# juanmc2005/diart

Measured on AMD Instinct MI355X. Metric: real-time-factor xRT streams/GPU @500ms step, higher is better.
Workload: dtype f16x3

## Files before the change

### diart_amd/build.py

```python
from __future__ import annotations

import os
import shutil
import subprocess
import sys
from concurrent.futures import ThreadPoolExecutor
from pathlib import Path

HERE = Path(__file__).resolve().parent
CSRC = HERE / "csrc"
LIB = HERE / "libdiart_amd.so"
LIB_EXPERIMENTS = HERE / "libdiart_amd_exp.so"
SOURCES = ["api.hip", "seg_api.hip", "xvec_api.hip", "kernel_api.hip", "ecapa_api.hip", "k_front.hip", "k_convgemm.hip", "k_gemm_f32.hip", "k_gemm_split.hip", "k_gemm_pre.hip",
           "k_mlp_head.hip", "k_conv_pool.hip", "k_lstm.hip", "k_lstm_mfma.hip", "k_pool.hip",
           "k_ecapa.hip", "ecm_api.hip", "k_ecapa_mel.hip", "sbx_api.hip", "titanet_api.hip", "k_titanet.hip", "sbr_api.hip", "k_sb_resnet.hip", "wespeaker_api.hip", "k_wespeaker.hip", "k_conv2d.hip", "k_resample.hip", "k_volume.hip", "k_rows_repeat.hip", "k_gather.hip", "resample_api.hip", "ring.hip", "cluster.cpp", "tail.cpp", "hostpool.cpp", "filebatch.cpp", "k_tune.hip", "k_tune_vad.hip", "k_tune_score.hip", "tune_score.cpp"]
EXPERIMENT_SOURCES = ["experiments/k_gemm_g2.hip", "experiments/k_gemm_g3.hip"]
ARCH = "gfx950"
EXTRA_FLAGS = {"k_lstm_mfma.hip": ["-fno-slp-vectorize"]}


def _hipcc() -> str:
    for cand in (os.environ.get("HIPCC"), shutil.which("hipcc"), "/opt/rocm/bin/hipcc"):
        if cand and Path(cand).exists():
            return cand
    raise RuntimeError("hipcc not found (set HIPCC)")


def _stale(out: Path, deps) -> bool:
    if not out.exists():
        return True
    t = out.stat().st_mtime
    return any(Path(d).stat().st_mtime > t for d in deps)


def build(force: bool = False, verbose: bool = False, experiments: bool = False) -> Path:
    hipcc = _hipcc()
    objdir = HERE / "build" / ("exp" if experiments else "ship")
    objdir.mkdir(parents=True, exist_ok=True)
    headers = [CSRC / "dz_common.h", CSRC / "dz_embed.h", CSRC / "dz_sincnet.h", CSRC / "hostpool.h", CSRC / "tune_core.h", CSRC / "clu_core.h", HERE.parent / "include" / "diart_amd.h",
               HERE.parent / "include" / "diart_amd_experiments.h"]
    flags = ["-O3", "-std=c++17", "-fPIC", f"--offload-arch={ARCH}", "-Wall", "-Wno-unused-function", f"-I{CSRC}"]
    sources, lib = list(SOURCES), LIB
    if experiments:
        flags.append("-DDZ_EXPERIMENTS")
        sources, lib = sources + EXPERIMENT_SOURCES, LIB_EXPERIMENTS

    def compile_one(src: str) -> Path:
        s = CSRC / src
        o = objdir / (s.stem + ".o")
        if force or _stale(o, [s, *headers]):
            cmd = [hipcc, *flags, *EXTRA_FLAGS.get(src, []), "-x", "hip", "-c", str(s), "-o", str(o)]
            r = subprocess.run(cmd, capture_output=True, text=True)
            if r.returncode != 0:
                raise RuntimeError(f"hipcc failed on {src}:\n{r.stderr}")
            if verbose and r.stderr.strip():
                print(r.stderr, file=sys.stderr)
        return o

    with ThreadPoolExecutor(max_workers=min(len(sources), os.cpu_count() or 4)) as ex:
        objs = list(ex.map(compile_one, sources))
    if force or _stale(lib, objs):
        cmd = [hipcc, "-shared", "-fPIC", f"--offload-arch={ARCH}", *map(str, objs), "-o", str(lib), "-lpthread"]
        r = subprocess.run(cmd, capture_output=True, text=True)
        if r.returncode != 0:
            raise RuntimeError(f"link failed:\n{r.stderr}")
    return lib


if __name__ == "__main__":
    print(build(force="--force" in sys.argv, verbose=True, experiments="--experiments" in sys.argv))
```

### diart_amd/csrc/dz_common.h

```cpp
#pragma once
#include <hip/hip_runtime.h>
#include <hip/hip_ext.h>
#include <stdint.h>
#include <stddef.h>
#include <mutex>
#include "../../include/diart_amd.h"

#ifdef DZ_EXPERIMENTS
#include <stdlib.h>
static inline const char* dz_exp_env(const char* name) { return getenv(name); }
#else
#define dz_exp_env(name) ((const char*)nullptr)
#endif
enum { DZ_OPT_F32_GEMM = 0, DZ_OPT_POOL_FUSE, DZ_OPT_PACK_CACHE, DZ_OPT_COUNT };
int dz_option(int id);

typedef float f32x4 __attribute__((ext_vector_type(4)));
typedef float f32x2 __attribute__((ext_vector_type(2)));

#define DZ_MFMA(a, b, c) __builtin_amdgcn_mfma_f32_16x16x4f32((a), (b), (c), 0, 0, 0)

#define DZ_LEAKY_SLOPE 0.01f

struct DzAttrOnce {
    std::mutex mu;
    bool done[64] = {};
    hipError_t raise(const void* fn, int bytes) {
        int d = 0;
        (void)hipGetDevice(&d);
        std::lock_guard<std::mutex> lk(mu);
        if (d >= 0 && d < 64 && done[d]) return hipSuccess;
        const hipError_t e = hipFuncSetAttribute(fn, hipFuncAttributeMaxDynamicSharedMemorySize, bytes);
        if (e == hipSuccess && d >= 0 && d < 64) done[d] = true;
        return e;
    }
};

struct DzLaunchProf {
    hipEvent_t start, stop;
};
struct DzProfScope {
    DzProfScope(int tag, int units);
    ~DzProfScope();
};
enum DzProfTag {
    DZ_T_WAVE = 0, DZ_T_CONV0, DZ_T_FIN, DZ_T_CONV1, DZ_T_CONV2, DZ_T_PROJ, DZ_T_REC, DZ_T_MLP, DZ_T_CLS,
    DZ_T_TDNN1, DZ_T_TDNN2, DZ_T_TDNN3, DZ_T_TDNN4, DZ_T_TDNN5, DZ_T_POOL, DZ_T_EMBLIN, DZ_T_L2, DZ_T_OSP, DZ_T_PSET,
    DZ_T_CDIST, DZ_T_PROJ0,
    DZ_T_ECAPA_FBANK, DZ_T_ECAPA_BLOCK0, DZ_T_ECAPA_WIDE, DZ_T_ECAPA_RES2, DZ_T_ECAPA_SE, DZ_T_ECAPA_ASP, DZ_T_ECAPA_FC,
    DZ_T_CONV0_PAIR, DZ_T_NSPLIT, DZ_T_COUNT
};
extern thread_local int* dz_cur_oflag;
struct DzRangeScope {
    int* prev;
    explicit DzRangeScope(int* f) : prev(dz_cur_oflag) { dz_cur_oflag = f; }
    ~DzRangeScope() { dz_cur_oflag = prev; }
};
extern thread_local DzLaunchProf* dz_launch_prof;
#define DZ_LAUNCH(kernel, grid, block, lds, st, ...)                                          \
    do {                                                                                      \
        if (dz_launch_prof) {                                                                 \
            hipExtLaunchKernelGGL(kernel, grid, block, lds, st, dz_launch_prof->start,        \
                                  dz_launch_prof->stop, 0, __VA_ARGS__);                      \
            dz_launch_prof = nullptr;                             \
        } else {                                                                              \
            hipLaunchKernelGGL(kernel, grid, block, lds, st, __VA_ARGS__);                    \
        }                                                                                     \
    } while (0)

__device__ __forceinline__ void dz_tile_map_lin(int L, int gx, int gy, int gz, int agroup, int& bx, int& by,
                                                int& bz) {
    const int NA = gx * gz, NA8 = NA & ~7;
    int a;
    if (L < NA8 * gy) {
        const int xcd = L & 7, j = L >> 3;
        const int per = NA8 >> 3;
        const int AG = agroup > 0 ? agroup : 4;
        const int g = j / (AG * gy), r = j - g * (AG * gy);
        const int gsz = per - g * AG < AG ? per - g * AG : AG;
        by = r / gsz;
        a = (g * AG + (r - by * gsz)) * 8 + xcd;
    } else {
        const int r = L - NA8 * gy;
        a = NA8 + r / gy;
        by = r - (r / gy) * gy;
    }
    bz = a / gx;
    bx = a - bz * gx;
}
__device__ __forceinline__ void dz_tile_map(int agroup, int& bx, int& by, int& bz) {
    const int gx = gridDim.x, gy = gridDim.y;
    dz_tile_map_lin(blockIdx.x + gx * (blockIdx.y + gy * blockIdx.z), gx, gy, gridDim.z, agroup, bx, by, bz);
}

__device__ __forceinline__ int dz_xcd_contiguous(int b, int grid) {
    return (grid & 7) == 0 ? (b & 7) * (grid >> 3) + (b >> 3) : b;
}

__host__ __device__ __forceinline__ long long dz_kb(long long row, int col, long long R) {
    return ((long long)(col >> 5) * R + row) * 32 + (col & 31);
}

__device__ __forceinline__ unsigned short* dz_split_base(void* ysplit, long long yplane, bool odd) {
    unsigned short* y = reinterpret_cast<unsigned short*>(ysplit);
    return odd ? y + (yplane - 1) : y;
}
__device__ __forceinline__ void dz_store_split(unsigned short* ypl, long long idx, float v, bool store,
                                               bool odd, float& amax) {
    amax = fmaxf(amax, fabsf(v));
    const float x = __builtin_amdgcn_fmed3f(v, -65504.f, 65504.f);
    const _Float16 h = (_Float16)x;
    const _Float16 lw = (_Float16)((x - (float)h) * 2048.f);
    const unsigned P = (unsigned)__builtin_bit_cast(unsigned short, h) |
                       ((unsigned)__builtin_bit_cast(unsigned short, lw) << 16);
    const unsigned Q = (unsigned)__builtin_amdgcn_update_dpp(0, (int)P, 0xB1, 0xF, 0xF, true);
    const unsigned word = odd ? ((Q >> 16) | (P & 0xffff0000u)) : ((P & 0xffffu) | (Q << 16));
    if (store) *reinterpret_cast<unsigned*>(ypl + idx) = word;
}

__device__ __forceinline__ void dz_norm_from_partials(const float* __restrict__ partials, int b, int ntile,
                                                      int C, int T, const float* __restrict__ gamma,
                                                      const float* __restrict__ beta, float* out, int tid,
                                                      int nthreads, double* scratch) {
    const int G = nthreads / C > 0 ? nthreads / C : 1;
    const int c = tid % C, g = tid / C;
    if (g < G) {
        double s = 0.0, ss = 0.0;
        const float2* pp = reinterpret_cast<const float2*>(partials) + ((long long)b * ntile * C + c);
        int t = g;
        for (; t + 3 * G < ntile; t += 4 * G) {
            const float2 a0 = pp[(long long)t * C], a1 = pp[(long long)(t + G) * C];
            const float2 a2 = pp[(long long)(t + 2 * G) * C], a3 = pp[(long long)(t + 3 * G) * C];
            s += (double)a0.x; ss += (double)a0.y;
            s += (double)a1.x; ss += (double)a1.y;
            s += (double)a2.x; ss += (double)a2.y;
            s += (double)a3.x; ss += (double)a3.y;
        }
        for (; t < ntile; t += G) {
            const float2 a = pp[(long long)t * C];
            s += (double)a.x; ss += (double)a.y;
        }
        scratch[(g * C + c) * 2] = s;
        scratch[(g * C + c) * 2 + 1] = ss;
    }
    __syncthreads();
    if (tid < C) {
        double s = 0.0, ss = 0.0;
        for (int k = 0; k < G; ++k) {
            s += scratch[(k * C + tid) * 2];
            ss += scratch[(k * C + tid) * 2 + 1];
        }
        const double mean = s / T;
        double var = ss / T - mean * mean;
        if (var < 0.0) var = 0.0;
        const double rstd = 1.0 / sqrt(var + 1e-5);
        const double sc = (double)gamma[tid] * rstd;
        out[tid] = (float)sc;
        out[C + tid] = (float)((double)beta[tid] - mean * sc);
    }
}

__device__ __forceinline__ void dz_flag_range(int* oflag, float amax) {
    if (oflag && amax > 65504.f) *oflag = 1;
}

void dz_set_error(const char* fmt, ...);
#define DZ_HIP(expr)                                                                     \
    do {                                                                                 \
        hipError_t _e = (expr);                                                          \
        if (_e != hipSuccess) {                                                          \
            dz_set_error("%s failed: %s (%s:%d)", #expr, hipGetErrorString(_e), __FILE__, \
                         __LINE__);                                                      \
            return 1;                                                                    \
        }                                                                                \
    } while (0)
#define DZ_REQUIRE(cond, ...)           \
    do {                                \
        if (!(cond)) {                  \
            dz_set_error(__VA_ARGS__);  \
            return 2;                   \
        }                               \
    } while (0)

struct Arena {
    char* base = nullptr;
    size_t used = 0;
    template <typename T = float>
    T* take(size_t n) {
        const size_t bytes = (n * sizeof(T) + 255) & ~size_t(255);
        T* p = base ? reinterpret_cast<T*>(base + used) : nullptr;
        used += bytes;
        return p;
    }
};

template <typename H>
int dz_arena_alloc(const char* who, H* h, void (*carve)(H*, Arena&)) {
    Arena a;
    carve(h, a);
    const hipError_t err = hipMalloc((void**)&h->arena, a.used);
    if (err != hipSuccess) {
        h->arena = nullptr;
        dz_set_error("%s: hipMalloc(%zu) failed: %s", who, a.used, hipGetErrorString(err));
        return 1;
    }
    DZ_HIP(hipMemset(h->arena, 0, a.used));
    a.base = h->arena;
    a.used = 0;
    carve(h, a);
    return 0;
}

inline int dz_check_rows_forward(const char* who, const void* h, int max_rows, const float* d_wave, long long wave_stride,
                                 const float* d_masks, int n, int mask_frames, const float* d_out,
                                 const char* frames = "mask_frames") {
    DZ_REQUIRE(h && d_wave && d_out, "%s: NULL argument", who);
    DZ_REQUIRE(n >= 1 && n <= max_rows, "%s: %d rows outside [1, %d]", who, n, max_rows);
    DZ_REQUIRE(d_masks == nullptr || mask_frames >= 1, "%s: %s %d", who, frames, mask_frames);
    DZ_REQUIRE(wave_stride >= 0, "%s: negative stride", who);
    return 0;
}
inline int dz_check_groups_forward(const char* who, const void* h, int max_rows, const float* d_wave,
                                   long long wave_stride, const float* d_masks, int n_groups, int rows_per_group,
                                   int mask_frames, const float* d_out) {
    DZ_REQUIRE(h && d_wave && d_masks && d_out, "%s: NULL argument", who);
    DZ_REQUIRE(n_groups >= 1 && rows_per_group >= 1 && (long long)n_groups * rows_per_group <= max_rows,
               "%s: %d groups x %d rows outside [1, %d]", who, n_groups, rows_per_group, max_rows);
    DZ_REQUIRE(mask_frames >= 1, "%s: mask_frames %d", who, mask_frames);
    DZ_REQUIRE(wave_stride >= 0, "%s: negative stride", who);
    return 0;
}

struct DzRowGeometry {
    int S, Tc, min_samples, hop;
    long long lstride;
    float* sig;
    int *lens, *nvalid, *nmask, *tooshort;
    int *tdev, *rep_nvalid, *rep_nmask, *rep_T;
    void init(int num_samples, int min_num_samples, int hop = 160, int window = 400);
    void carve(Arena& a, size_t rows);
    int prologue(const float* d_wave, long long wave_stride, const float* d_masks, int mask_frames, int G, int K,
                 int rows_per_wave, hipStream_t st);
};

#define DZ_WS_G 8
__device__ __forceinline__ bool dz_ws_bad(const float* __restrict__ mom, int b) {
    const unsigned* m = reinterpret_cast<const unsigned*>(mom) + (long long)b * 2 * DZ_WS_G;
    bool bad = false;
#pragma unroll
    for (int i = 0; i < DZ_WS_G; ++i) bad |= (m[2 * i] & 0x7f800000u) == 0x7f800000u;
    return bad;
}
#ifdef DZ_EXPERIMENTS
extern long long* dz_conv_pool_dbg;
#endif
int dz_launch_wave_stats(const float* wave, long long stride, int B, int S, float* mom,
                         hipStream_t st);
int dz_launch_wave_stats_combine(const float* mom, int B, int S, float* stats, hipStream_t st);
int dz_launch_sinc_conv0(const float* wave, long long stride, int B, int S, const float* stats,
                         int stats_are_moments, float gamma, float beta, const float* filt,
                         float* y0, int P0, float* partials, int ntile, hipStream_t st);
int dz_launch_sinc_conv0_split(const float* wave, long long stride, int B, int S, const float* stats,
                               int stats_are_moments, float gamma, float beta, const void* filt_split,
                               float* y0, int P0, float* partials, int ntile, hipStream_t st, const void* ffrag = nullptr);
int dz_sinc_bank_frag_bytes();
int dz_launch_sinc_bank_frag(const void* fsp, void* frag, hipStream_t st);
int dz_conv0_split_ntile(int F0);
int dz_launch_sinc_conv0_pair(const float* wave, long long stride, int B, int S, const float* moments,
                              const void* pair_planes, const float* pair_bsum, float gamma_seg, float gamma_emb,
                              float* y0_seg, float* y0_emb, int P0, float* part_seg, float* part_emb, int ntile,
                              hipStream_t st);
int dz_launch_finalize_norm(const float* partials, int B, int ntile, int C, int T,
                            const float* gamma, const float* beta, float* scale, float* shift,
                            hipStream_t st);

typedef dz_convgemm_desc DzConvGemm;
constexpr int DZ_EPI_TG = 0x100;
int dz_launch_convgemm(const DzConvGemm& p, hipStream_t st);
bool dz_gemm_f32_ok(const DzConvGemm& p);
int dz_launch_gemm_f32(const DzConvGemm& p, hipStream_t st);
int dz_launch_gemm_split(const DzConvGemm& p, hipStream_t st);
int dz_launch_norm_f32(const float* y, const float* part, int ntile, int P, const float* gamma, const float* beta,
                       float* out, int B, hipStream_t st);
int dz_launch_norm_split(const float* y, const float* part, int ntile, int P, const float* gamma, const float* beta,
                         void* planes, long long plane, int B, hipStream_t st);
int dz_launch_conv_pool(const DzConvGemm& p, hipStream_t st, const void* wfrag = nullptr);
int dz_conv_pool_wfrag_bytes(int Cin);
int dz_launch_conv_pool_wfrag(int Cin, const void* wsplit, int Kpad, void* out, hipStream_t st);
int dz_launch_gemm_pre(const DzConvGemm& p, hipStream_t st);
#ifdef DZ_EXPERIMENTS
int dz_launch_gemm_g2(const DzConvGemm& p, int mt, hipStream_t st);
int dz_g2_default_mt();
#endif
int dz_gemm_gen();
#ifdef DZ_EXPERIMENTS
int dz_launch_gemm_g3(const DzConvGemm& p, int mt, hipStream_t st);
int dz_g3_error(int reset);
#endif
__device__ __forceinline__ float dz_pool_weight(const float* wr, int Fw, int T, int t) {
    const int F = Fw < 0 ? -Fw : Fw;
    if (F == T) return wr[t];
    const float scale = (float)F / (float)T;
    if (Fw < 0) {
        int i = (int)floorf((float)t * scale);
        if (i > F - 1) i = F - 1;
        return wr[i];
    }
    float src = scale * ((float)t + 0.5f) - 0.5f;
    if (src < 0.f) src = 0.f;
    const int i0 = (int)src;
    const int i1 = i0 + (i0 < F - 1 ? 1 : 0);
    const float l1 = src - (float)i0;
    return (1.f - l1) * wr[i0] + l1 * wr[i1];
}

struct DzPoolFuse {
    const float* w;
    int Fw, K;
    int P, T;
    int np;
    float* part;
    float* s0;
};
inline int dz_pool_pieces(int P) { return (P + 2 * 128 - 2) / 128; }
bool dz_gemm_pre_pool_ok(const DzConvGemm& p);
int dz_launch_gemm_pre_pool(const DzConvGemm& p, const DzPoolFuse& q, hipStream_t st);
int dz_launch_pool_combine(const float* part, const float* s0, int nx, int K, int np, int P, int T, int C,
                           int Npad, float* out, int ldo, hipStream_t st);
int dz_convgemm_ntile(int Tout);

int dz_launch_lstm(const float* gx, const float* whh, float* hout, void* hsplit, long long hplane,
                   int B, int T, int unit_major, hipStream_t st);
int dz_launch_lstm_mfma(const float* gx, const void* whh_split, float* hout, void* hsplit,
                        long long hplane, int B, int T, int unit_major, int variant, hipStream_t st);

int dz_launch_stats_pool(const float* X, long long xstride, int T, int C, int ldx,
                         const float* weights, int Fw, int rows, int rows_per_x, float* out, int ldo,
                         hipStream_t st);
int dz_launch_osp(const float* seg, int B, int F, int K, float gamma, float beta, int normalize,
                  int speaker_major, float* out, hipStream_t st);
__device__ __forceinline__ float dz_powg(float x, float gamma) {
    if (gamma == 3.f) return (x * x) * x;
    if (gamma == 2.f) return x * x;
    if (gamma == 1.f) return x;
    return powf(x, gamma);
}
__device__ __forceinline__ void dz_seg_decide(const float* lg, int classes, int K, int powerset, float* s) {
    if (powerset) {
        int best = 0;
        float bv = lg[0];
        for (int c = 1; c < classes; ++c)
            if (lg[c] > bv) {
                bv = lg[c];
                best = c;
            }
        int a = -1, b2 = -1;
        if (best >= 1 && best <= K) {
            a = best - 1;
        } else if (best > K) {
            int idx = best - K - 1;
            for (int i = 0; i < K && a < 0; ++i) {
                const int cnt = K - 1 - i;
                if (idx < cnt) {
                    a = i;
                    b2 = i + 1 + idx;
                } else {
                    idx -= cnt;
                }
            }
        }
        for (int k = 0; k < K; ++k) s[k] = (k == a || k == b2) ? 1.f : 0.f;
    } else {
        for (int k = 0; k < K; ++k) s[k] = 1.f / (1.f + expf(-lg[k]));
    }
}
__device__ __forceinline__ float dz_vad_frame(const float* s, int K) {
    float m = s[0];
    for (int k = 1; k < K; ++k) m = (s[k] > m || s[k] != s[k]) ? s[k] : m;
    return m;
}
__device__ __forceinline__ void dz_osp_frame(const float* s, int K, float gamma, float beta, float* w) {
    float e[8], m = -INFINITY;
    for (int k = 0; k < K; ++k) m = fmaxf(m, beta * s[k]);
    float sum = 0.f;
    for (int k = 0; k < K; ++k) {
        e[k] = expf(beta * s[k] - m);
        sum += e[k];
    }
    for (int k = 0; k < K; ++k) {
        const float pr = e[k] / sum;
        float wv = dz_powg(s[k], gamma) * dz_powg(pr, gamma);
        if (wv < 1e-8f) wv = 1e-8f;
        w[k] = wv;
    }
}

int dz_launch_seg_head(const float* m1, const float* cw, const float* cb, int B, int F, int classes, int K,
                       int powerset, float* seg, float gamma, float beta, int normalize, float* wout,
                       hipStream_t st, const float* wave_mom = nullptr, float* vad = nullptr);
struct DzMlpHead {
    const void* Xsplit;
    long long xplane;
    const void *W0split, *W1split;
    const float *b0, *b1, *cw, *cb;
    int rows, F, classes, K, powerset;
    float gamma, beta;
    float* seg;
    float* wout;
    int* oflag;
    const float* wave_mom;
    float* vad;
};
int dz_launch_mlp_head(const DzMlpHead& p, hipStream_t st);
int dz_launch_l2norm(float* x, int rows, int dim, float norm, hipStream_t st);
int dz_launch_splitk_finish(const float* parts, int nsplit, long long stride, int rows, int dim,
                            int normalize, float* out, hipStream_t st, const float* wave_mom = nullptr,
                            int rows_per_x = 1);
int dz_launch_powerset(const float* logp, int rows, int classes, int speakers, float* out,
                       hipStream_t st);
int dz_launch_cdist(const float* emb, const double* centers, int n, int k, int g, int dim,
                    double* out, hipStream_t st);

int dz_launch_mask_compact(const float* wave, long long stride, int S, const float* masks, int Fw,
                           int rows, float* sig, long long sig_stride, int* lens, hipStream_t st,
                           int rows_per_wave = 1);
int dz_launch_ecapa_geometry(const int* lens, int G, int K, int Tc, int min_samples, int hop, int* nvalid,
                             int* nmask, int* tooshort, int* tdev, int* rv, int* rm, int* rt, hipStream_t st);
int dz_launch_power(const float* spec, int lds, int bins, long long rows, float* pw, hipStream_t st);
int dz_launch_fbank_post(const float* melp, int n_mels, int T, int rows, const int* nvalid, float* feats,
                         hipStream_t st, const int* tdev = nullptr);
int dz_launch_se_mean(const float* x, int T, int C, int ldx, int rows, const int* nmask, float* s,
                      hipStream_t st);
int dz_launch_se_apply(const float* x, int ldx, const float* gate, const float* resid, int ldr,
                       float* out, int ldo, int rows, int T, int C, hipStream_t st);
int dz_launch_se_apply_planes(const float* x, int ldx, const float* gate, const float* resid, int ldr, float* out,
                              int ldo, void* planes, long long plane, int rows, int T, int C, hipStream_t st);
int dz_launch_asp_gstats(const float* x, int T, int C, int rows, const int* nmask, float* g,
                         hipStream_t st);
int dz_launch_asp_pool(const float* x, const float* logit, int T, int C, int rows, const int* nmask,
                       float* pooled, hipStream_t st);
int dz_launch_nan_rows(float* out, int rows, int dim, const int* flags, hipStream_t st);
int dz_launch_sb_stats_pool(const float* x, int T, int C, int ldx, int rows, const int* nvalid, float mean_bias,
                            float std_bias, float* pooled, hipStream_t st);

int dz_launch_ecm_prep(const float* sig, long long sig_stride, const int* lens, int rows, int K, float* csig,
                       long long cstride, int* lmax_out, hipStream_t st);
int dz_launch_ecm_magnitude(const float* spec, long long rows, float* mag, hipStream_t st);
int dz_launch_ecm_post(const float* melp, int T, int rows, const int* nvalid, float* feats, hipStream_t st);

struct DzConv2d {
    const float* X;
    const float* W;
    const void* Wsplit;
    const float* bias;
    const float* R;
    float* Y;
    int B, Fi, Ti, Cin, Fo, To, Cout, taps, stride, relu;
    int* oflag;
    const int* ext;
};
inline DzConv2d dz_conv2d(const float* W, const void* Wsplit, const float* bias, const float* X, int B, int Fi, int Ti,
                          int Cin, int Cout, int taps, int stride, const float* R, int relu, const int* ext, float* Y) {
    DzConv2d p = {};
    p.X = X; p.W = W; p.Wsplit = Wsplit; p.bias = bias; p.R = R; p.Y = Y; p.ext = ext;
    p.B = B; p.Fi = Fi; p.Ti = Ti; p.Cin = Cin; p.Cout = Cout; p.taps = taps; p.stride = stride; p.relu = relu;
    p.Fo = stride >= 1 ? (Fi - 1) / stride + 1 : 0;
    p.To = stride >= 1 ? (Ti - 1) / stride + 1 : 0;
    return p;
}
int dz_launch_conv2d(const DzConv2d& p, hipStream_t st);

enum { DZ_SBR_SE_SLICES = 16 };
int dz_launch_sbr_extents(const int* tdev, int rows, int s0, int s1, int s2, int s3, int* ext, hipStream_t st);
int dz_launch_sbr_stem(const float* feats, int rows, int Tb, int F, int C, const float* w, const float* b,
                       const int* ext, float* y, hipStream_t st);
int dz_launch_sbr_se_sum(const float* y, int rows, int Tb, int F, int C, const int* ext, float* part, hipStream_t st);
int dz_launch_sbr_se_fc(const float* part, int rows, int F, int C, int Cr, const int* ext, const float* w1t,
                        const float* b1, const float* w2t, const float* b2, float* gate, hipStream_t st);
int dz_launch_sbr_se_apply(const float* y, const float* gate, const float* r, int rows, int Tb, int F, int C,
                           const int* ext, float* out, hipStream_t st);
int dz_launch_sbr_att_pool(const float* x, const float* logits, int ldl, int rows, int Tb, int C, const int* ext,
                           float* pooled, hipStream_t st);

int dz_launch_wsp_fbank(const float* wave, long long stride, int N, int T, const float* mel, float* raw, int* bad,
                        hipStream_t st);
int dz_launch_wsp_cmn(const float* raw, int N, int T, const int* bad, float* feats, hipStream_t st);
int dz_launch_wsp_conv1(const float* feats, int N, int T, const float* w, const float* b, float* y, hipStream_t st);
int dz_launch_wsp_pool(const float* x, int B, int T4, const float* weights, int Fw, int K, const int* bad,
                       float* out, int* rflag, hipStream_t st);

int dz_launch_resample(const float* in, long long in_stride, long long in_len, int rows, const float* table,
                       int tap_major, int n, int n_pad, int o, int width, int T, float* out, long long out_stride,
                       long long out_len, hipStream_t st);

int dz_launch_rows_repeat(const float* wave, long long stride, int n_rows, int S, int* differs, int* repeat_out,
                          hipStream_t st);

struct dz_ctx {
    int device;
    int* oflag_host;
    int* oflag_dev;
    void* conv0_frag;
    void* convp_frag;
    const void* conv0_src;
    const void* convp_src;
    int convp_cin, convp_kpad;
    std::mutex frag_mu;
    hipStream_t conv0_user, convp_user;
    bool conv0_used, convp_used;
    int* rr_flags;
    int rr_cap;
    int* rr_host;
    int* rr_dev;
    std::mutex rr_mu;
    hipStream_t rr_user;
    bool rr_dirty;
};
```

### diart_amd/csrc/dz_embed.h

```cpp
#pragma once
#include "dz_common.h"

#include <string.h>
#include <new>

inline bool dz_conv_pool_enabled() {
    const char* v = dz_exp_env("DZ_CONV_POOL");
    return !(v && v[0] == '0');
}

struct DzGemm {
    DzConvGemm p;
    const void *wsplit, *wfrag;
    int tag, units;

    static DzGemm dense(const dz_layer& L, const float* X, int ldx, long long rows, int Cin, float* Y, int ldy,
                        int Nstore, int epi) {
        return conv1d(L, X, ldx, 1, (int)rows, Cin, Y, ldy, Nstore, epi).xstride(0, 0);
    }
    static DzGemm conv1d(const dz_layer& L, const float* X, int ldx, int B, int T, int Cin, float* Y, int ldy,
                         int Nstore, int epi) {
        DzGemm g;
        memset(&g, 0, sizeof(g));
        g.wsplit = L.wsplit;
        g.tag = -1;
        DzConvGemm& p = g.p;
        p.X = X; p.W = L.w; p.bias = L.b; p.e0 = L.s; p.e1 = L.h; p.Y = Y;
        p.B = B; p.Tin = p.Tout = p.Tstore = T; p.Cin = Cin; p.taps = 1; p.dil = 1; p.K = p.Kpad = Cin;
        p.Npad = p.Nstore = Nstore; p.ldx = ldx; p.ldy = ldy; p.epi = epi;
        return g.xstride((long long)T * ldx, (long long)T * ldy);
    }
    DzGemm& xstride(long long xbs, long long ybs) { p.xbs = xbs; p.ybs = ybs; return *this; }
    DzGemm& taps(int n, int dil, int pad) {
        p.taps = n; p.dil = dil; p.pad = pad; p.K = n * p.Cin;
        p.Tout = p.Tstore = pad ? p.Tin : p.Tin - (n - 1) * dil;
        return *this;
    }
    DzGemm& padded(int Kpad, int Npad) { p.Kpad = Kpad; p.Npad = Npad; return *this; }
    DzGemm& x2(const float* X2) { p.X2 = X2; return *this; }
    DzGemm& rowbias(const float* rb) { p.rowbias = rb; return *this; }
    DzGemm& splitk(int n, long long ysplit) { p.ksplit = n; p.ysplit = ysplit; return *this; }
    DzGemm& xplanes(const void* Xs, long long xplane) { p.Xsplit = Xs; p.xplane = Xs ? xplane : 0; return *this; }
    DzGemm& planes_out(void* Ys, long long yplane) { p.Ysplit = Ys; p.yplane = Ys ? yplane : 0; return *this; }
    DzGemm& norm_partials(const float* part, int tiles, int T, const float* gamma, const float* beta, int nld) {
        p.npart = part; p.npart_tiles = tiles; p.npart_T = T; p.ngamma = gamma; p.nbeta = beta;
        p.nld = nld; p.norm_on_load = 1;
        return *this;
    }
    DzGemm& norm_scaled(const float* nscale, const float* nshift, int nld) {
        p.nscale = nscale; p.nshift = nshift; p.nld = nld; p.norm_on_load = 1;
        return *this;
    }
    DzGemm& pool3(float* partials) {
        p.partials = partials; p.Tstore = p.Tout / 3; p.ybs = (long long)p.Tstore * p.ldy;
        return *this;
    }
    DzGemm& frag(const void* f) { wfrag = f; return *this; }
    DzGemm& tdev(const int* T) { p.Tdev = T; return *this; }
    DzGemm& prof(int t, int u) { tag = t; units = u; return *this; }

    int run(hipStream_t st) {
        DzProfScope ps(tag, units);
        if (p.Xsplit) {
            p.X = p.W = nullptr;
            p.Wsplit = wsplit;
            return dz_launch_gemm_pre(p, st);
        }
        if (wsplit && p.ksplit <= 1) {
            p.Wsplit = wsplit;
            if (p.epi == DZ_EPI_POOL3)
                return dz_conv_pool_enabled() ? dz_launch_conv_pool(p, st, wfrag) : dz_launch_gemm_split(p, st);
            p.Npad = (p.Npad + 127) / 128 * 128;
            return dz_launch_gemm_split(p, st);
        }
        DZ_REQUIRE(p.Ysplit == nullptr, "DzGemm: plane output asked of a layer that is not on the split-f16 path");
        return dz_launch_convgemm(p, st);
    }
    int run_pooled(const DzPoolFuse& q, hipStream_t st) {
        DzProfScope ps(tag, units);
        p.X = p.W = nullptr;
        p.Wsplit = wsplit;
        return dz_launch_gemm_pre_pool(p, q, st);
    }
};

constexpr int DZ_TAG_OF_GEMM = -2;
inline int dz_splitk_linear(const dz_layer& L, const float* X, int rows, int Cin, int Kpad, int N, int nsplit,
                            float* parts, int finish, float* out, hipStream_t st, int tag = -1,
                            int finish_tag = DZ_TAG_OF_GEMM, const float* wave_mom = nullptr, int rows_per_x = 1) {
    const long long ysplit = (long long)rows * N;
    if (int rc = DzGemm::dense(L, X, Cin, rows, Cin, parts, N, N, DZ_EPI_BIAS).padded(Kpad, N).splitk(nsplit, ysplit)
                     .prof(tag, rows / rows_per_x).run(st))
        return rc;
    DzProfScope ps(finish_tag == DZ_TAG_OF_GEMM ? tag : finish_tag, rows / rows_per_x);
    return dz_launch_splitk_finish(parts, nsplit, ysplit, rows, N, finish, out, st, wave_mom, rows_per_x);
}

inline int dz_fbank_front(const dz_layer& dft, const dz_layer& mel, const float* sig, long long lstride, int N, int T,
                          float* spec, float* pw, int nmel, int mel_npad, float* melp, hipStream_t st, int tag = -1) {
    const long long NT = (long long)N * T;
    int rc;
    if ((rc = DzGemm::conv1d(dft, sig, 160, N, T, 400, spec, 404, 402, DZ_EPI_BIAS).xstride(lstride, (long long)T * 404)
                  .padded(416, 448).prof(tag, N).run(st)))
        return rc;
    { DzProfScope ps(tag, N); if ((rc = dz_launch_power(spec, 404, 201, NT, pw, st))) return rc; }
    return DzGemm::dense(mel, pw, 204, NT, 204, melp, nmel, nmel, DZ_EPI_BIAS).padded(224, mel_npad).prof(tag, N).run(st);
}

struct DzAspTail {
    const float *wms, *zeros;
    const dz_layer *tdnn, *conv, *fc;
    float *gstat, *rb, *a1, *logits, *pooled, *parts;
    int nsplit, tag_asp, tag_fc;
};
inline int dz_asp_tail(const DzAspTail& a, const float* x, int N, int T, int C, int emb, const int* frames, float* out,
                       hipStream_t st) {
    int rc;
    { DzProfScope ps(a.tag_asp, N); if ((rc = dz_launch_asp_gstats(x, T, C, N, frames, a.gstat, st))) return rc; }
    const dz_layer wms = {a.wms, a.zeros, nullptr, nullptr, nullptr};
    if ((rc = dz_splitk_linear(wms, a.gstat, N, 2 * C, 2 * C, 128, a.nsplit, a.parts, 0, a.rb, st, a.tag_asp))) return rc;
    if ((rc = DzGemm::conv1d(*a.tdnn, x, C, N, T, C, a.a1, 128, 128, DZ_EPI_RELU_BN_TANH).rowbias(a.rb)
                  .prof(a.tag_asp, N).run(st)))
        return rc;
    if ((rc = DzGemm::dense(*a.conv, a.a1, 128, (long long)N * T, 128, a.logits, C, C, DZ_EPI_BIAS).prof(a.tag_asp, N)
                  .run(st)))
        return rc;
    { DzProfScope ps(a.tag_asp, N); if ((rc = dz_launch_asp_pool(x, a.logits, T, C, N, frames, a.pooled, st))) return rc; }
    return dz_splitk_linear(*a.fc, a.pooled, N, 2 * C, 2 * C, emb, a.nsplit, a.parts, 0, out, st, a.tag_fc);
}

struct DzEcapaTrunk {
    float *feats, *b0, *t1, *res, *t2, *cat, *mfa, *a1;
    float *smean, *sfc1, *gate, *gstat, *rb, *pooled, *parts;
    unsigned short *b0s, *ress, *cats;
    void carve(Arena& a, size_t N, size_t Tc, bool split);
    int run(const dz_ecapa_weights& w, int N, int T, const int* nmask, const int* tdev, float* d_out,
            hipStream_t st) const;
};

template <typename H>
int dz_handle_destroy(H* h) {
    if (h) {
        if (h->arena) (void)hipFree(h->arena);
        delete h;
    }
    return 0;
}
template <typename H, typename W>
int dz_handle_create(const char* who, dz_ctx* ctx, const W* w, int max_rows, int num_samples, int min_samples,
                     void (*carve)(H*, Arena&), H** out, int hop = 160, int window = 400) {
    DZ_REQUIRE(ctx && w && out, "%s: NULL argument", who);
    DZ_REQUIRE(max_rows >= 1 && num_samples >= min_samples, "%s: max_rows %d, %d samples", who, max_rows, num_samples);
    DZ_HIP(hipSetDevice(ctx->device));
    H* h = new (std::nothrow) H;
    DZ_REQUIRE(h != nullptr, "%s: out of memory", who);
    memset(h, 0, sizeof(*h));
    h->ctx = ctx; h->w = *w; h->Nm = max_rows;
    h->geo.init(num_samples, min_samples, hop, window);
    if (int rc = dz_arena_alloc(who, h, carve)) {
        dz_handle_destroy(h);
        return rc;
    }
    *out = h;
    return 0;
}
template <typename H, typename Run>
int dz_handle_forward(const char* who, H* h, const float* d_wave, long long wave_stride, const float* d_masks, int N,
                      int mask_frames, float* d_out, void* stream, Run run) {
    if (int rc = dz_check_rows_forward(who, h, h ? h->Nm : 0, d_wave, wave_stride, d_masks, N, mask_frames, d_out))
        return rc;
    DZ_HIP(hipSetDevice(h->ctx->device));
    DzRangeScope range_scope(h->ctx->oflag_dev);
    return run(h, d_wave, wave_stride, d_masks, 1, N, 1, mask_frames, 0, d_out, (hipStream_t)stream);
}
template <typename H, typename Run>
int dz_handle_forward_groups(const char* who, H* h, const float* d_wave, long long wave_stride, const float* d_masks,
                             int n_groups, int rows_per_group, int mask_frames, int normalize, float* d_out,
                             void* stream, Run run) {
    if (int rc = dz_check_groups_forward(who, h, h ? h->Nm : 0, d_wave, wave_stride, d_masks, n_groups, rows_per_group,
                                         mask_frames, d_out))
        return rc;
    DZ_HIP(hipSetDevice(h->ctx->device));
    DzRangeScope range_scope(h->ctx->oflag_dev);
    return run(h, d_wave, wave_stride, d_masks, n_groups, rows_per_group, rows_per_group, mask_frames, normalize, d_out,
               (hipStream_t)stream);
}
```

### diart_amd/csrc/k_gemm_pre.hip

```cpp
#include "dz_common.h"
#include <stdlib.h>
#include <type_traits>

namespace {

typedef _Float16 f16x8 __attribute__((ext_vector_type(8)));
typedef _Float16 f16x2 __attribute__((ext_vector_type(2)));
typedef float f32x16 __attribute__((ext_vector_type(16)));

constexpr int BM = 128, BN = 128, KT = 32;
constexpr int PLANE_B = 128 * 64;
constexpr int plane_a(int MW) { return 64 * MW * 64; }
constexpr int stage_bytes(int MW) { return 2 * plane_a(MW) + 2 * PLANE_B; }
constexpr size_t lds_bytes(int MW) { return 2 * (size_t)stage_bytes(MW) + 3 * BN * sizeof(float); }
constexpr int MW_BIG = 6;
constexpr float LO_UNSCALE = 1.f / 2048.f;

__device__ __forceinline__ float leaky(float v) { return fmaxf(v, v * DZ_LEAKY_SLOPE); }

constexpr int YT_PITCH = 132;
constexpr int POOL_PAR = BM * YT_PITCH * 4;
constexpr int POOL_WT = POOL_PAR + 3 * BN * 4;
constexpr int POOL_RED = POOL_WT + 4 * BM * 4;
constexpr int POOL_S0 = POOL_RED + 2 * 2 * 4 * BN * 4;
constexpr size_t POOL_LDS = POOL_S0 + 8 * 8 * 2 * 4 + 8 * 2 * 4;

template <int EPI, int MW, int MT, int NT, bool ILV = false, bool POOL = false>
__device__ __forceinline__ void gemm_pre_tile(const DzConvGemm& p, const int t0, const int n0, char* smem,
                                              const int flags = 0, const DzPoolFuse* q = nullptr) {
    constexpr int PLANE_A = plane_a(MW), STAGE = stage_bytes(MW), PAR_OFF = POOL ? POOL_PAR : 2 * STAGE;
    static_assert(!POOL || (MW == 2 && MT == 2 && NT == 2), "pooled epilogue: 128 x 128 tiles only");
    const int tid = threadIdx.x;
    const int w = __builtin_amdgcn_readfirstlane(tid >> 6), l = tid & 63;

    constexpr int PA = 2 * MT * MW, PB = 4 * NT, NWAVE = 2 * MW;
    constexpr int NWA = (NWAVE * PA + (PA + PB) / 2) / (PA + PB);
    constexpr int JMAX_A = (2 * PA + NWA - 1) / NWA, JMAX_B = (2 * PB + (NWAVE - NWA) - 1) / (NWAVE - NWA);
    constexpr int JMAX = JMAX_A > JMAX_B ? JMAX_A : JMAX_B;
    const bool isB = w >= NWA;
    const int rank = isB ? w - NWA : w, group = isB ? NWAVE - NWA : NWA, npc = isB ? PB : PA;
    const unsigned short* src = isB ? reinterpret_cast<const unsigned short*>(p.Wsplit)
                                    : reinterpret_cast<const unsigned short*>(p.Xsplit);
    const int prows = isB ? p.Npad : (int)((unsigned)p.xplane / (unsigned)p.ldx);
    const long long plane_el = isB ? (long long)p.Npad * p.Kpad : p.xplane;
    const unsigned nbytes = (unsigned)((long long)prows * (isB ? p.Kpad : p.ldx) * 2);
    const __amdgpu_buffer_rsrc_t rs_hi = __builtin_amdgcn_make_buffer_rsrc((void*)src, 0, nbytes, 0x00020000);
    const __amdgpu_buffer_rsrc_t rs_lo = __builtin_amdgcn_make_buffer_rsrc((void*)(src + plane_el), 0, nbytes, 0x00020000);
    const int voff0 = ((isB ? n0 : t0) + (l >> 2)) * 64 + (((l & 3) ^ ((l >> 4) & 3)) << 4);
    constexpr int vstep = 16 * 64;
    const int kb_bytes = prows * 64;
    const int dst0 = isB ? 2 * PLANE_A : 0, dplane = isB ? PLANE_B : PLANE_A;
    auto issue = [&](int kt, int stage) {
        int cblk = kt, tap = 0;
        if (p.taps > 1) {
            cblk = kt / p.taps;
            tap = kt - cblk * p.taps;
        }
        const int soff = isB ? (tap * (p.Cin >> 5) + cblk) * kb_bytes : cblk * kb_bytes + tap * p.dil * 64;
        char* dst = smem + stage * STAGE + dst0;
#pragma unroll
        for (int j = 0; j < JMAX; ++j) {
            const int q = rank + j * group;
            if (q >= 2 * npc) break;
            const int lo = q >= npc, i = q - lo * npc;
            __builtin_amdgcn_raw_ptr_buffer_load_lds(lo ? rs_lo : rs_hi,
                (__attribute__((address_space(3))) void*)(dst + lo * dplane + i * 1024), 16,
                voff0 + i * vstep, soff, 0, 0);
        }
    };

    const int li = l & 31, g = l >> 5;
    const int wm = w >> 1, wn = w & 1;
    const int sw = (li >> 2) & 3;
    int foff[2];
#pragma unroll
    for (int ks = 0; ks < 2; ++ks) foff[ks] = li * 64 + (((2 * ks + g) ^ sw) << 4);
    f32x16 accm[MT][NT], accx[MT][NT];
#pragma unroll
    for (int mt = 0; mt < MT; ++mt)
#pragma unroll
        for (int nt = 0; nt < NT; ++nt)
#pragma unroll
            for (int r = 0; r < 16; ++r) accm[mt][nt][r] = accx[mt][nt][r] = 0.f;

    auto compute = [&](int stage) {
        const char* st = smem + stage * STAGE;
        const char* sa = st + (wm * 32 * MT) * 64;
        const char* sb = st + 2 * PLANE_A + (wn * 32 * NT) * 64;
#pragma unroll
        for (int ks = 0; ks < 2; ++ks) {
            f16x8 ah[MT], al[MT], bh[NT], bl[NT];
#pragma unroll
            for (int t = 0; t < MT; ++t) {
                ah[t] = *reinterpret_cast<const f16x8*>(sa + t * 2048 + foff[ks]);
                al[t] = *reinterpret_cast<const f16x8*>(sa + PLANE_A + t * 2048 + foff[ks]);
            }
#pragma unroll
            for (int t = 0; t < NT; ++t) {
                bh[t] = *reinterpret_cast<const f16x8*>(sb + t * 2048 + foff[ks]);
                bl[t] = *reinterpret_cast<const f16x8*>(sb + PLANE_B + t * 2048 + foff[ks]);
            }
#pragma unroll
            for (int mt = 0; mt < MT; ++mt)
#pragma unroll
                for (int nt = 0; nt < NT; ++nt) {
                    accx[mt][nt] = __builtin_amdgcn_mfma_f32_32x32x16_f16(bh[nt], al[mt], accx[mt][nt], 0, 0, 0);
                    accm[mt][nt] = __builtin_amdgcn_mfma_f32_32x32x16_f16(bh[nt], ah[mt], accm[mt][nt], 0, 0, 0);
                    accx[mt][nt] = __builtin_amdgcn_mfma_f32_32x32x16_f16(bl[nt], ah[mt], accx[mt][nt], 0, 0, 0);
                }
        }
    };

    const int nk = p.Kpad / KT;
    issue(0, 0);
    constexpr bool FULL = MW == 2 && MT == 2 && NT == 2;
    float* par = reinterpret_cast<float*>(smem + PAR_OFF);
    {
        constexpr bool AFF = EPI == DZ_EPI_TDNN || EPI == DZ_EPI_RELU_BN;
        const int which = tid >> 5, c4 = (tid & 31) * 4;
        if (which < (AFF ? 3 : 1)) {
            const float* src = which == 0 ? p.bias : which == 1 ? p.e0 : p.e1;
            f32x4 v = {0.f, 0.f, 0.f, 0.f};
            if (n0 + c4 + 3 < p.Npad) v = *reinterpret_cast<const f32x4*>(src + n0 + c4);
            *reinterpret_cast<f32x4*>(par + which * BN + c4) = v;
        }
    }
    if (FULL && ILV) {
        const int r2 = w & 1;
        char* const dbase = smem + dst0 + r2 * 1024;
        const int vofs = voff0 + r2 * vstep;
        int cblk = 0, tap = 0;
        const int tap_step = isB ? (p.Cin >> 5) * kb_bytes : p.dil * 64;
        auto advance = [&]() -> int {
            if (++tap == p.taps) { tap = 0; ++cblk; }
            return cblk * kb_bytes + tap * tap_step;
        };
        int soff_next = 0, stage_next = 0;
        const bool no_dma = flags & 2, no_rd = flags & 4;
        const bool skip_a = (flags & 32) && !isB;
        auto piece = [&](int j) {
            const int lo = j >= 4, i = r2 + 2 * (j & 3);
            (void)i;
            if (no_dma || (skip_a && tap != 0 && cblk > 0)) return;
            __builtin_amdgcn_raw_ptr_buffer_load_lds(lo ? rs_lo : rs_hi,
                (__attribute__((address_space(3))) void*)(dbase + stage_next * STAGE + lo * dplane + (j & 3) * 2048), 16,
                vofs + (j & 3) * 2 * vstep, soff_next, 0, 0);
        };
        const char* sa0 = smem + (wm * 64) * 64;
        const char* sb0 = smem + 2 * PLANE_A + (wn * 64) * 64;
#define DZ_RD(base, plane, t, ks) (*reinterpret_cast<const f16x8*>((no_rd ? smem : (base) + (plane) + (t) * 2048) + foff[ks]))
#define DZ_MM(mt, nt)                                                                                     \
    accx[mt][nt] = __builtin_amdgcn_mfma_f32_32x32x16_f16(bh[nt], al[mt], accx[mt][nt], 0, 0, 0);          \
    accm[mt][nt] = __builtin_amdgcn_mfma_f32_32x32x16_f16(bh[nt], ah[mt], accm[mt][nt], 0, 0, 0);          \
    accx[mt][nt] = __builtin_amdgcn_mfma_f32_32x32x16_f16(bl[nt], ah[mt], accx[mt][nt], 0, 0, 0)
#define DZ_PIN() __builtin_amdgcn_sched_barrier(0)
        auto body = [&](const int kt, auto more_c) {
            constexpr bool more = decltype(more_c)::value;
            asm volatile("s_waitcnt vmcnt(0) lgkmcnt(0)\n\ts_barrier" ::: "memory");
            soff_next = advance();
            stage_next = (kt + 1) & 1;
            const char* sa = sa0 + (kt & 1) * STAGE;
            const char* sb = sb0 + (kt & 1) * STAGE;
            f16x8 ah[2], al[2], bh[2], bl[2];
            bh[0] = DZ_RD(sb, 0, 0, 0); al[0] = DZ_RD(sa, PLANE_A, 0, 0); ah[0] = DZ_RD(sa, 0, 0, 0);
            bl[0] = DZ_RD(sb, PLANE_B, 0, 0);
            bh[1] = DZ_RD(sb, 0, 1, 0); bl[1] = DZ_RD(sb, PLANE_B, 1, 0);
            ah[1] = DZ_RD(sa, 0, 1, 0); al[1] = DZ_RD(sa, PLANE_A, 1, 0);
            DZ_PIN();
            accx[0][0] = __builtin_amdgcn_mfma_f32_32x32x16_f16(bh[0], al[0], accx[0][0], 0, 0, 0);
            accm[0][0] = __builtin_amdgcn_mfma_f32_32x32x16_f16(bh[0], ah[0], accm[0][0], 0, 0, 0);
            DZ_PIN();
            if (more) piece(0);
            DZ_PIN();
            accx[0][0] = __builtin_amdgcn_mfma_f32_32x32x16_f16(bl[0], ah[0], accx[0][0], 0, 0, 0);
            accx[0][1] = __builtin_amdgcn_mfma_f32_32x32x16_f16(bh[1], al[0], accx[0][1], 0, 0, 0);
            DZ_PIN();
            if (more) piece(1);
            DZ_PIN();
            accm[0][1] = __builtin_amdgcn_mfma_f32_32x32x16_f16(bh[1], ah[0], accm[0][1], 0, 0, 0);
            accx[0][1] = __builtin_amdgcn_mfma_f32_32x32x16_f16(bl[1], ah[0], accx[0][1], 0, 0, 0);
            DZ_PIN();
            if (more) piece(2);
            ah[0] = DZ_RD(sa, 0, 0, 1); al[0] = DZ_RD(sa, PLANE_A, 0, 1);
            DZ_PIN();
            accx[1][1] = __builtin_amdgcn_mfma_f32_32x32x16_f16(bh[1], al[1], accx[1][1], 0, 0, 0);
            accm[1][1] = __builtin_amdgcn_mfma_f32_32x32x16_f16(bh[1], ah[1], accm[1][1], 0, 0, 0);
            DZ_PIN();
            if (more) piece(3);
            DZ_PIN();
            accx[1][1] = __builtin_amdgcn_mfma_f32_32x32x16_f16(bl[1], ah[1], accx[1][1], 0, 0, 0);
            accx[1][0] = __builtin_amdgcn_mfma_f32_32x32x16_f16(bh[0], al[1], accx[1][0], 0, 0, 0);
            DZ_PIN();
            if (more) piece(4);
            bh[1] = DZ_RD(sb, 0, 1, 1); bl[1] = DZ_RD(sb, PLANE_B, 1, 1);
            DZ_PIN();
            accm[1][0] = __builtin_amdgcn_mfma_f32_32x32x16_f16(bh[0], ah[1], accm[1][0], 0, 0, 0);
            accx[1][0] = __builtin_amdgcn_mfma_f32_32x32x16_f16(bl[0], ah[1], accx[1][0], 0, 0, 0);
            DZ_PIN();
            if (more) piece(5);
            bh[0] = DZ_RD(sb, 0, 0, 1); bl[0] = DZ_RD(sb, PLANE_B, 0, 1);
            ah[1] = DZ_RD(sa, 0, 1, 1); al[1] = DZ_RD(sa, PLANE_A, 1, 1);
            DZ_PIN();
            accx[0][1] = __builtin_amdgcn_mfma_f32_32x32x16_f16(bh[1], al[0], accx[0][1], 0, 0, 0);
            accm[0][1] = __builtin_amdgcn_mfma_f32_32x32x16_f16(bh[1], ah[0], accm[0][1], 0, 0, 0);
            DZ_PIN();
            if (more) piece(6);
            DZ_PIN();
            accx[0][1] = __builtin_amdgcn_mfma_f32_32x32x16_f16(bl[1], ah[0], accx[0][1], 0, 0, 0);
            accx[0][0] = __builtin_amdgcn_mfma_f32_32x32x16_f16(bh[0], al[0], accx[0][0], 0, 0, 0);
            DZ_PIN();
            if (more) piece(7);
            DZ_PIN();
            accm[0][0] = __builtin_amdgcn_mfma_f32_32x32x16_f16(bh[0], ah[0], accm[0][0], 0, 0, 0);
            accx[0][0] = __builtin_amdgcn_mfma_f32_32x32x16_f16(bl[0], ah[0], accx[0][0], 0, 0, 0);
            DZ_MM(1, 0);
            DZ_MM(1, 1);
        };
        for (int kt = 0; kt + 1 < nk; ++kt) body(kt, std::true_type{});
        body(nk - 1, std::false_type{});
#undef DZ_RD
#undef DZ_MM
#undef DZ_PIN
    } else
    for (int kt = 0; kt < nk; ++kt) {
        asm volatile("s_waitcnt vmcnt(0) lgkmcnt(0)\n\ts_barrier" ::: "memory");
        if (kt + 1 < nk) issue(kt + 1, (kt + 1) & 1);
        compute(kt & 1);
    }

    typedef _Float16 f16x4 __attribute__((ext_vector_type(4)));
    unsigned short* Yhi = reinterpret_cast<unsigned short*>(p.Ysplit);
    const long long yrows = Yhi ? (long long)((unsigned)p.yplane / (unsigned)p.ldy) : 0;
    float amax = 0.f;
    float* yt = reinterpret_cast<float*>(smem);
    if (POOL) __syncthreads();
    if constexpr (!POOL) {
        const bool whole = n0 + 64 * NT <= p.Nstore;
        const long long ybytes = Yhi ? 2 * (long long)yrows * p.ldy : 4 * (long long)p.Tout * p.ldy;
        if (whole && (Yhi != nullptr) != (p.Y != nullptr) && ybytes < (1ll << 31) && !(flags & 64)) {
            const unsigned nrec = __builtin_amdgcn_readfirstlane((unsigned)ybytes);
            const __amdgpu_buffer_rsrc_t r0 = __builtin_amdgcn_make_buffer_rsrc(Yhi ? (void*)Yhi : (void*)p.Y, 0, nrec, 0x00020000);
            const __amdgpu_buffer_rsrc_t r1 = __builtin_amdgcn_make_buffer_rsrc(Yhi ? (void*)(Yhi + p.yplane) : (void*)p.Y, 0, nrec, 0x00020000);
            typedef unsigned u32x2 __attribute__((ext_vector_type(2)));
            typedef unsigned u32x4 __attribute__((ext_vector_type(4)));
            const float* parl = par + wn * 32 * NT + 4 * g;
            auto sweep = [&](auto kind_c) {
                constexpr int KIND = decltype(kind_c)::value;
                constexpr bool PL = KIND != 0;
                u32x2 ph = {0u, 0u}, pw = {0u, 0u};
#pragma unroll
            for (int mt = 0; mt < MT; ++mt) {
                const int t = t0 + wm * 32 * MT + mt * 32 + li;
                const bool ok = t < p.Tout;
                float am = 0.f;
                const int vo = !ok ? (int)0x80000000 : KIND == 2 ? t * 64 + 16 * g : KIND == 1 ? t * 64 + 8 * g : (t * p.ldy + 4 * g) * 4;
#pragma unroll
                for (int nt = 0; nt < NT; ++nt) {
                    const int cb = n0 + wn * 32 * NT + nt * 32;
                    const int so = __builtin_amdgcn_readfirstlane(PL ? (cb >> 5) * (int)yrows * 64 : cb * 4);
#pragma unroll
                    for (int k = 0; k < 4; ++k) {
                        asm volatile("" ::: "memory");
                        const float* pg = parl + nt * 32 + 8 * k;
                        const f32x4 bv = *reinterpret_cast<const f32x4*>(pg);
                        f32x4 e0 = {1.f, 1.f, 1.f, 1.f}, e1 = {0.f, 0.f, 0.f, 0.f};
                        if (EPI == DZ_EPI_TDNN || EPI == DZ_EPI_RELU_BN) {
                            e0 = *reinterpret_cast<const f32x4*>(pg + BN);
                            e1 = *reinterpret_cast<const f32x4*>(pg + 2 * BN);
                        }
                        f32x4 v;
#pragma unroll
                        for (int e = 0; e < 4; ++e) {
                            float x = (accm[mt][nt][4 * k + e] + accx[mt][nt][4 * k + e] * LO_UNSCALE) + bv[e];
                            if (EPI == DZ_EPI_BIAS_LEAKY) x = leaky(x);
                            if (EPI == DZ_EPI_TDNN) x = leaky(x) * e0[e] + e1[e];
                            if (EPI == DZ_EPI_RELU_BN) x = fmaxf(x, 0.f) * e0[e] + e1[e];
                            v[e] = x;
                        }
                        if constexpr (!PL) {
                            __builtin_amdgcn_raw_buffer_store_b128(__builtin_bit_cast(u32x4, v), r0, vo + 32 * k, so, 0);
                        } else {
#pragma unroll
                        for (int e = 0; e < 4; ++e) {
                            am = fmaxf(am, fabsf(v[e]));
                            v[e] = __builtin_amdgcn_fmed3f(v[e], -65504.f, 65504.f);
                        }
                        asm volatile("" : "+v"(am));
                        const f16x4 hi = __builtin_convertvector(v, f16x4);
                        const f16x4 lo = __builtin_convertvector((v - __builtin_convertvector(hi, f32x4)) * 2048.f, f16x4);
                        if constexpr (KIND == 1) {
                            __builtin_amdgcn_raw_buffer_store_b64(__builtin_bit_cast(u32x2, hi), r0, vo + 16 * k, so, 0);
                            __builtin_amdgcn_raw_buffer_store_b64(__builtin_bit_cast(u32x2, lo), r1, vo + 16 * k, so, 0);
                        } else if ((k & 1) == 0) {
                            ph = __builtin_bit_cast(u32x2, hi);
                            pw = __builtin_bit_cast(u32x2, lo);
                        } else {
                            const u32x2 ch = __builtin_bit_cast(u32x2, hi), cw = __builtin_bit_cast(u32x2, lo);
                            u32x4 oh, ow;
#pragma unroll
                            for (int d = 0; d < 2; ++d) {
                                const auto sh = __builtin_amdgcn_permlane32_swap(ph[d], ch[d], false, false);
                                const auto sw2 = __builtin_amdgcn_permlane32_swap(pw[d], cw[d], false, false);
                                oh[d] = sh[0]; oh[2 + d] = sh[1];
                                ow[d] = sw2[0]; ow[2 + d] = sw2[1];
                            }
                            __builtin_amdgcn_raw_buffer_store_b128(oh, r0, vo + 32 * (k >> 1), so, 0);
                            __builtin_amdgcn_raw_buffer_store_b128(ow, r1, vo + 32 * (k >> 1), so, 0);
                        }
                        }
                    }
                }
                if (ok) amax = fmaxf(amax, am);
            }
            };
            if (!Yhi) sweep(std::integral_constant<int, 0>{});
            else if (flags & 128) sweep(std::integral_constant<int, 1>{});
            else sweep(std::integral_constant<int, 2>{});
            dz_flag_range(p.oflag, amax);
            return;
        }
    }
#pragma unroll
    for (int mt = 0; mt < MT; ++mt) {
        const int t = t0 + wm * 32 * MT + mt * 32 + li;
        const bool ok = t < p.Tout;
#pragma unroll
        for (int nt = 0; nt < NT; ++nt)
#pragma unroll
            for (int k = 0; k < 4; ++k) {
                asm volatile("" ::: "memory");
                const int n = n0 + wn * 32 * NT + nt * 32 + 8 * k + 4 * g;
                const int nc = n - n0;
                const f32x4 bv = *reinterpret_cast<const f32x4*>(par + nc);
                f32x4 e0 = {1.f, 1.f, 1.f, 1.f}, e1 = {0.f, 0.f, 0.f, 0.f};
                if (EPI == DZ_EPI_TDNN || EPI == DZ_EPI_RELU_BN) {
                    e0 = *reinterpret_cast<const f32x4*>(par + BN + nc);
                    e1 = *reinterpret_cast<const f32x4*>(par + 2 * BN + nc);
                }
                f32x4 v;
#pragma unroll
                for (int e = 0; e < 4; ++e) {
                    float x = (accm[mt][nt][4 * k + e] + accx[mt][nt][4 * k + e] * LO_UNSCALE) + bv[e];
                    if (EPI == DZ_EPI_BIAS_LEAKY) x = leaky(x);
                    if (EPI == DZ_EPI_TDNN) x = leaky(x) * e0[e] + e1[e];
                    if (EPI == DZ_EPI_RELU_BN) x = fmaxf(x, 0.f) * e0[e] + e1[e];
                    v[e] = x;
                }
                if (POOL) {
                    if (!(flags & 16)) *reinterpret_cast<f32x4*>(yt + (t - t0) * YT_PITCH + nc) = v;
                    continue;
                }
                const long long idx = (long long)t * p.ldy + n;
                if (p.Y && ok) {
                    if (n + 3 < p.Nstore) {
                        *reinterpret_cast<f32x4*>(p.Y + idx) = v;
                    } else {
#pragma unroll
                        for (int e = 0; e < 4; ++e)
                            if (n + e < p.Nstore) p.Y[idx + e] = v[e];
                    }
                }
                if (Yhi) {
#pragma unroll
                    for (int e = 0; e < 4; ++e) {
                        if (n + e >= p.Nstore) v[e] = 0.f;
                        if (ok) amax = fmaxf(amax, fabsf(v[e]));
                        v[e] = __builtin_amdgcn_fmed3f(v[e], -65504.f, 65504.f);
                    }
                    const f16x4 hi = __builtin_convertvector(v, f16x4);
                    const f16x4 lo = __builtin_convertvector((v - __builtin_convertvector(hi, f32x4)) * 2048.f, f16x4);
                    if (ok) {
                        const long long kidx = dz_kb(t, n, yrows);
                        *reinterpret_cast<f16x4*>(Yhi + kidx) = hi;
                        *reinterpret_cast<f16x4*>(Yhi + p.yplane + kidx) = lo;
                    }
                }
            }
    }
    dz_flag_range(p.oflag, amax);
    if constexpr (POOL) {
        if (flags & 24) return;
        float* wt = reinterpret_cast<float*>(smem + POOL_WT);
        float* red = reinterpret_cast<float*>(smem + POOL_RED);
        float* s0t = reinterpret_cast<float*>(smem + POOL_S0);
        float* s0f = s0t + 8 * 8 * 2;
        const int K = q->K, P = q->P, T = q->T;
        for (int i = tid; i < 4 * BM; i += 256) {
            const int rl = i >> 2, k = i & 3, r = t0 + rl;
            const int b = r / P, t = r - b * P;
            float wv = 0.f;
            if (k < K && t < T && r < p.Tout) {
                wv = 1.f;
                if (q->w) wv = dz_pool_weight(q->w + (long long)(b * K + k) * (q->Fw < 0 ? -q->Fw : q->Fw), q->Fw, T, t);
            }
            wt[i] = wv;
        }
        __syncthreads();
        const int b0 = t0 / P;
        int rb = (b0 + 1) * P - t0;
        if (rb > BM) rb = BM;
        if (tid < 64) {
            const int pk = tid >> 3, sub = tid & 7, part = pk >> 2, k = pk & 3;
            float a = 0.f, a2 = 0.f;
            if (k < K) {
                const int lo = max(part ? rb : 0, 16 * sub), hi = min(part ? BM : rb, 16 * sub + 16);
                for (int r = lo; r < hi; ++r) {
                    const float wv = wt[4 * r + k];
                    a += wv;
                    a2 += wv * wv;
                }
            }
            s0t[(pk * 8 + sub) * 2] = a;
            s0t[(pk * 8 + sub) * 2 + 1] = a2;
        }
        __syncthreads();
        if (tid < 8) {
            float a = 0.f, a2 = 0.f;
            for (int sub = 0; sub < 8; ++sub) {
                a += s0t[(tid * 8 + sub) * 2];
                a2 += s0t[(tid * 8 + sub) * 2 + 1];
            }
            s0f[tid * 2] = a;
            s0f[tid * 2 + 1] = a2;
        }
        const int wv_ = tid >> 6, c2 = 2 * (tid & 63);
        const int nx = p.Tout / P;
        auto pool_part = [&](auto kk_tag, const int part) {
            constexpr int KK = decltype(kk_tag)::value;
            const int lo = max(part ? rb : 0, 32 * wv_), hi = min(part ? BM : rb, 32 * wv_ + 32);
            float S[KK][2];
#pragma unroll
            for (int k = 0; k < KK; ++k) S[k][0] = S[k][1] = 0.f;
#pragma unroll 4
            for (int r = lo; r < hi; ++r) {
                const f32x2 x = *reinterpret_cast<const f32x2*>(yt + r * YT_PITCH + c2);
                const f32x4 w4 = *reinterpret_cast<const f32x4*>(wt + 4 * r);
#pragma unroll
                for (int k = 0; k < KK; ++k) {
                    S[k][0] = __builtin_fmaf(w4[k], x[0], S[k][0]);
                    S[k][1] = __builtin_fmaf(w4[k], x[1], S[k][1]);
                }
            }
#pragma unroll
            for (int k = 0; k < KK; ++k)
                *reinterpret_cast<f32x2*>(red + (wv_ * 4 + k) * BN + c2) = (f32x2){S[k][0], S[k][1]};
            __syncthreads();
            float mean[KK][2];
#pragma unroll
            for (int k = 0; k < KK; ++k) {
                f32x2 a = {0.f, 0.f};
#pragma unroll
                for (int v = 0; v < 4; ++v) a += *reinterpret_cast<const f32x2*>(red + (v * 4 + k) * BN + c2);
                const float v1 = s0f[(part * 4 + k) * 2];
                mean[k][0] = v1 > 0.f ? a[0] / v1 : 0.f;
                mean[k][1] = v1 > 0.f ? a[1] / v1 : 0.f;
            }
            __syncthreads();
#pragma unroll
            for (int k = 0; k < KK; ++k) S[k][0] = S[k][1] = 0.f;
#pragma unroll 4
            for (int r = lo; r < hi; ++r) {
                const f32x2 x = *reinterpret_cast<const f32x2*>(yt + r * YT_PITCH + c2);
                const f32x4 w4 = *reinterpret_cast<const f32x4*>(wt + 4 * r);
#pragma unroll
                for (int k = 0; k < KK; ++k) {
                    const float d0 = x[0] - mean[k][0], d1 = x[1] - mean[k][1];
                    S[k][0] = __builtin_fmaf(w4[k] * d0, d0, S[k][0]);
                    S[k][1] = __builtin_fmaf(w4[k] * d1, d1, S[k][1]);
                }
            }
#pragma unroll
            for (int k = 0; k < KK; ++k)
                *reinterpret_cast<f32x2*>(red + (wv_ * 4 + k) * BN + c2) = (f32x2){S[k][0], S[k][1]};
            __syncthreads();
            const int b = b0 + part;
            if (wv_ == 0 && b < nx) {
                const int piece = t0 / BM - (b * P) / BM;
#pragma unroll
                for (int k = 0; k < KK; ++k) {
                    f32x2 m2 = {0.f, 0.f};
#pragma unroll
                    for (int v = 0; v < 4; ++v) m2 += *reinterpret_cast<const f32x2*>(red + (v * 4 + k) * BN + c2);
                    float* o = q->part + ((((long long)b * q->np + piece) * K + k) * p.Npad + n0 + c2) * 2;
                    *reinterpret_cast<f32x4*>(o) = (f32x4){mean[k][0], m2[0], mean[k][1], m2[1]};
                    if (n0 == 0 && c2 == 0) {
                        float* so = q->s0 + (((long long)b * q->np + piece) * K + k) * 2;
                        so[0] = s0f[(part * 4 + k) * 2];
                        so[1] = s0f[(part * 4 + k) * 2 + 1];
                    }
                }
            }
        };
        for (int part = 0; part < (rb < BM ? 2 : 1); ++part) {
            if (part) __syncthreads();
            switch (K) {
                case 1: pool_part(std::integral_constant<int, 1>{}, part); break;
                case 2: pool_part(std::integral_constant<int, 2>{}, part); break;
                case 3: pool_part(std::integral_constant<int, 3>{}, part); break;
                default: pool_part(std::integral_constant<int, 4>{}, part); break;
            }
        }
    }
}

template <int EPI, bool ILV>
__global__ __launch_bounds__(256, 2) void gemm_pre_kernel(DzConvGemm p, int mbig, int msmall, int flags) {
    extern __shared__ __attribute__((aligned(16))) char smem[];
#ifndef DZ_EXPERIMENTS
    flags = 0;
#endif
    const int gy = p.Npad / BN, L = blockIdx.x;
    if (L < mbig * gy) {
        int bx, by, bz;
        dz_tile_map_lin(L, mbig, gy, 1, p.agroup, bx, by, bz);
        gemm_pre_tile<EPI, 2, 2, 2, ILV>(p, bx * BM, by * BN, smem, flags);
    } else {
        const int Ls = L - mbig * gy, gys = 2 * gy;
        const int xcd = Ls & 7, j = Ls >> 3;
        const int ms = (j / gys) * 8 + xcd, by = j % gys;
        if (ms >= msmall) return;
        gemm_pre_tile<EPI, 2, 1, 1>(p, mbig * BM + ms * 64, by * 64, smem);
    }
}

__global__ __launch_bounds__(256, 2) void gemm_pre_pool_kernel(DzConvGemm p, DzPoolFuse q, int gx, int flags) {
    extern __shared__ __attribute__((aligned(16))) char smem[];
    const int gy = p.Npad / BN;
    int bx, by, bz;
    dz_tile_map_lin(blockIdx.x, gx, gy, 1, p.agroup, bx, by, bz);
#ifndef DZ_EXPERIMENTS
    flags = 0;
#endif
    gemm_pre_tile<DZ_EPI_TDNN, 2, 2, 2, true, true>(p, bx * BM, by * BN, smem, flags, &q);
}

template <int EPI>
__global__ __launch_bounds__(64 * 2 * MW_BIG) void gemm_pre_big_kernel(DzConvGemm p) {
    extern __shared__ __attribute__((aligned(16))) char smem[];
    const int gy = p.Npad / BN, gx = (p.Tout + 64 * MW_BIG - 1) / (64 * MW_BIG);
    int bx, by, bz;
    dz_tile_map_lin(blockIdx.x, gx, gy, 1, p.agroup, bx, by, bz);
    gemm_pre_tile<EPI, MW_BIG, 2, 2>(p, bx * 64 * MW_BIG, by * BN, smem);
}
int big_tiles_mode() {
    static const int mode = [] {
        const char* e = dz_exp_env("DZ_GEMM_BIG");
        return e ? atoi(e) : 0;
    }();
    return mode;
}

bool interleaved_loop() {
    static const bool on = [] {
        const char* e = dz_exp_env("DZ_GP_LOOP");
        return !(e && e[0] == '0');
    }();
    return on;
}

int dbg_flags() {
    static const int f = [] {
        const char* e = dz_exp_env("DZ_GP_DBG");
        return e ? atoi(e) : 0;
    }();
    return f;
}

bool tail_tiles_enabled() {
    static const bool on = [] {
        const char* e = dz_exp_env("DZ_GEMM_TAIL");
        return e && e[0] == '1';
    }();
    return on;
}
int wg_slots() {
    static const int slots = [] {
        int dev = 0, cus = 256;
        if (hipGetDevice(&dev) == hipSuccess) hipDeviceGetAttribute(&cus, hipDeviceAttributeMultiprocessorCount, dev);
        return 2 * (cus > 0 ? cus : 256);
    }();
    return slots;
}

template <int EPI>
int launch(const DzConvGemm& p, hipStream_t st) {
    static DzAttrOnce attr_ilv;
    DZ_HIP(attr_ilv.raise((const void*)gemm_pre_kernel<EPI, true>, (int)lds_bytes(2)));
    const int gx = (p.Tout + BM - 1) / BM, gy = p.Npad / BN, slots = wg_slots();
#ifdef DZ_EXPERIMENTS
    static DzAttrOnce attr_once, attr_big;
    DZ_HIP(attr_once.raise((const void*)gemm_pre_kernel<EPI, false>, (int)lds_bytes(2)));
    {
        const int gxb = (p.Tout + 64 * MW_BIG - 1) / (64 * MW_BIG);
        const int mode = big_tiles_mode();
        if (mode == 1 && gxb >= 8) {
            DZ_HIP(attr_big.raise((const void*)gemm_pre_big_kernel<EPI>, (int)lds_bytes(MW_BIG)));
            DZ_LAUNCH((gemm_pre_big_kernel<EPI>), dim3(gxb * gy), dim3(64 * 2 * MW_BIG), lds_bytes(MW_BIG), st, p);
            DZ_HIP(hipGetLastError());
            return 0;
        }
    }
#endif
    int mbig = gx;
    const int tiles = gx * gy, rem = tiles % slots;
    if (4 * tiles < slots)
        mbig = 0;
    else if (tail_tiles_enabled() && rem != 0 && 4 * rem < 3 * slots)
        mbig = (tiles / slots) * slots / gy;
    const int rows_left = p.Tout - mbig * BM;
    const int msmall = rows_left > 0 ? (rows_left + 63) / 64 : 0;
    const int nwg = mbig * gy + ((msmall + 7) / 8) * 8 * (2 * gy);
#ifdef DZ_EXPERIMENTS
    if (!interleaved_loop())
        DZ_LAUNCH((gemm_pre_kernel<EPI, false>), dim3(nwg), dim3(256), lds_bytes(2), st, p, mbig, msmall, 0);
    else
#endif
        DZ_LAUNCH((gemm_pre_kernel<EPI, true>), dim3(nwg), dim3(256), lds_bytes(2), st, p, mbig, msmall, dbg_flags());
    DZ_HIP(hipGetLastError());
    return 0;
}

}

int dz_gemm_gen() {
    static const int gen = [] {
        const char* e = dz_exp_env("DZ_GEMM_GEN");
        const int v = e ? atoi(e) : 1;
        return v == 2 || v == 3 ? v : 1;
    }();
    return gen;
}

bool dz_gemm_pre_pool_ok(const DzConvGemm& p) {
    const int gx = (p.Tout + BM - 1) / BM, gy = p.Npad / BN;
    return 4 * gx * gy >= wg_slots();
}

int dz_launch_gemm_pre_pool(const DzConvGemm& p_in, const DzPoolFuse& q, hipStream_t st) {
    DzConvGemm p = p_in;
    if (!p.oflag) p.oflag = dz_cur_oflag;
    DZ_REQUIRE(p.Wsplit && p.Xsplit && q.part && q.s0, "gemm_pre_pool: NULL operand");
    DZ_REQUIRE(p.epi == DZ_EPI_TDNN && p.B == 1 && p.taps == 1 && p.K == p.Kpad && p.Cin % KT == 0 &&
                   p.Npad % BN == 0 && p.Tout == p.Tin,
               "gemm_pre_pool: built for the flattened 1 x 1 TDNN layer");
    DZ_REQUIRE(q.np == dz_pool_pieces(q.P), "gemm_pre_pool: np must be dz_pool_pieces(P)");
    DZ_REQUIRE(q.K >= 1 && q.K <= 4 && q.P >= BM && q.T >= 2 && q.T <= q.P && p.Tout % q.P == 0 && (q.Fw >= 2 || q.Fw <= -2),
               "gemm_pre_pool: 1..4 speakers, chunk pitch >= 128 rows (got K %d, P %d, T %d)", q.K, q.P, q.T);
    DZ_REQUIRE(p.ldx > 0 && p.ldx % KT == 0 && p.xplane % p.ldx == 0 && p.xplane / p.ldx >= p.Tin,
               "gemm_pre_pool: kb-major input planes need ldx %% 32 == 0 and xplane = rows * ldx with rows >= Tin");
    DZ_REQUIRE(p.xplane * 2 < (1ll << 31) && (long long)p.Npad * p.Kpad * 2 < (1ll << 31),
               "gemm_pre_pool: operand plane exceeds the 2 GiB buffer-offset range");
    static const int pool_ag = [] {
        const char* e = dz_exp_env("DZ_POOL_AG");
        return e && atoi(e) > 0 ? atoi(e) : 1;
    }();
    if (!p.agroup) p.agroup = pool_ag;
    static DzAttrOnce attr_once;
    DZ_HIP(attr_once.raise((const void*)gemm_pre_pool_kernel, (int)POOL_LDS));
    const int gx = (p.Tout + BM - 1) / BM, gy = p.Npad / BN;
    DZ_LAUNCH(gemm_pre_pool_kernel, dim3(gx * gy), dim3(256), POOL_LDS, st, p, q, gx, dbg_flags());
    DZ_HIP(hipGetLastError());
    return 0;
}

int dz_launch_gemm_pre(const DzConvGemm& p_in, hipStream_t st) {
    DzConvGemm p = p_in;
    if (!p.oflag) p.oflag = dz_cur_oflag;
    DZ_REQUIRE(p.Wsplit != nullptr && p.Xsplit != nullptr,
               "gemm_pre: Wsplit / Xsplit (f16 hi/lo planes of W and of the input) are NULL");
    DZ_REQUIRE(p.Y != nullptr || p.Ysplit != nullptr, "gemm_pre: no output");
    DZ_REQUIRE(p.B == 1, "gemm_pre: flattened layers only (B = 1)");
    DZ_REQUIRE(p.K == p.Kpad && p.K == p.taps * p.Cin && p.Cin % KT == 0,
               "gemm_pre: K = taps * Cin without padding, Cin a multiple of 32");
    DZ_REQUIRE(p.Npad % BN == 0, "gemm_pre: Npad must be a multiple of 128");
    DZ_REQUIRE(p.Tout > 0 && p.Tout == p.Tin - (p.taps - 1) * p.dil, "gemm_pre: Tout mismatch");
    DZ_REQUIRE(p.pad == 0 && p.X2 == nullptr && p.rowbias == nullptr && p.ksplit <= 1 && !p.norm_on_load,
               "gemm_pre: padding / second input / row bias / split-K / norm-on-load are not built here");
    DZ_REQUIRE(p.ldx > 0 && p.ldx % KT == 0 && p.xplane % p.ldx == 0 && p.xplane / p.ldx >= p.Tin,
               "gemm_pre: kb-major input planes need ldx %% 32 == 0 and xplane = rows * ldx with rows >= Tin");
    DZ_REQUIRE(p.xplane * 2 < (1ll << 31) && (long long)p.Npad * p.Kpad * 2 < (1ll << 31),
               "gemm_pre: operand plane exceeds the 2 GiB buffer-offset range");
    DZ_REQUIRE(p.Ysplit == nullptr || (p.ldy > 0 && p.ldy % KT == 0 && p.yplane % p.ldy == 0 && p.yplane / p.ldy >= p.Tout &&
                                       p.Npad <= p.ldy && p.yplane * 2 < (1ll << 31)),
               "gemm_pre: kb-major output planes need ldy %% 32 == 0, yplane = rows * ldy with rows >= Tout, Npad <= ldy");
    DZ_REQUIRE(p.Y == nullptr || (p.ldy % 4 == 0 && ((uintptr_t)p.Y & 15) == 0),
               "gemm_pre: f32 output needs ldy a multiple of 4 and a 16-byte aligned base");
#ifdef DZ_EXPERIMENTS
    if (dz_gemm_gen() >= 2 && 4 * ((p.Tout + BM - 1) / BM) * (p.Npad / BN) >= wg_slots()) {
        static const int g3_min_k = [] {
            const char* e = dz_exp_env("DZ_G3_MINK");
            return e ? atoi(e) : 1024;
        }();
        if (dz_gemm_gen() == 3) {
            if (p.K >= g3_min_k) return dz_launch_gemm_g3(p, 0, st);
        } else {
            return dz_launch_gemm_g2(p, 0, st);
        }
    }
#endif
    switch (p.epi) {
        case DZ_EPI_BIAS: return launch<DZ_EPI_BIAS>(p, st);
        case DZ_EPI_BIAS_LEAKY: return launch<DZ_EPI_BIAS_LEAKY>(p, st);
        case DZ_EPI_TDNN: return launch<DZ_EPI_TDNN>(p, st);
        case DZ_EPI_RELU_BN: return launch<DZ_EPI_RELU_BN>(p, st);
    }
    dz_set_error("gemm_pre: epilogue %d is not built on the pre-split path", p.epi);
    return 2;
}
```

### diart_amd/csrc/kernel_api.hip

```cpp
#include "dz_sincnet.h"

extern "C" int dz_k_convgemm(dz_ctx* ctx, const dz_convgemm_desc* d, void* stream) {
    DZ_REQUIRE(ctx && d, "dz_k_convgemm: NULL argument");
    DZ_HIP(hipSetDevice(ctx->device));
    DzRangeScope range_scope(ctx->oflag_dev);
    return dz_launch_convgemm(*d, (hipStream_t)stream);
}
extern "C" int dz_k_gemm_f32(dz_ctx* ctx, const dz_convgemm_desc* d, void* stream) {
    DZ_REQUIRE(ctx && d, "dz_k_gemm_f32: NULL argument");
    DZ_HIP(hipSetDevice(ctx->device));
    return dz_launch_gemm_f32(*d, (hipStream_t)stream);
}
extern "C" int dz_k_gemm_split(dz_ctx* ctx, const dz_convgemm_desc* d, void* stream) {
    DZ_REQUIRE(ctx && d, "dz_k_gemm_split: NULL argument");
    DZ_HIP(hipSetDevice(ctx->device));
    DzRangeScope range_scope(ctx->oflag_dev);
    return dz_launch_gemm_split(*d, (hipStream_t)stream);
}
extern "C" int dz_k_gemm_pre(dz_ctx* ctx, const dz_convgemm_desc* d, void* stream) {
    DZ_REQUIRE(ctx && d, "dz_k_gemm_pre: NULL argument");
    DZ_HIP(hipSetDevice(ctx->device));
    DzRangeScope range_scope(ctx->oflag_dev);
    return dz_launch_gemm_pre(*d, (hipStream_t)stream);
}
#ifdef DZ_EXPERIMENTS
static int gemm_gen_open(const char* who, dz_ctx* ctx, const dz_convgemm_desc* d, DzConvGemm* p) {
    DZ_REQUIRE(ctx && d, "%s: NULL argument", who);
    DZ_REQUIRE(d->Wsplit && d->Xsplit && (d->Y || d->Ysplit) && d->B == 1 && d->K == d->Kpad && d->K == d->taps * d->Cin &&
                   d->Cin % 32 == 0 && d->Npad % 128 == 0 && d->pad == 0 && !d->X2 && !d->rowbias && d->ksplit <= 1 &&
                   !d->norm_on_load && d->Tout > 0 && d->Tout == d->Tin - (d->taps - 1) * d->dil && d->ldx % 32 == 0 &&
                   d->xplane % d->ldx == 0 && d->xplane / d->ldx >= d->Tin,
               "%s: the requirements of dz_k_gemm_pre apply", who);
    DZ_HIP(hipSetDevice(ctx->device));
    *p = *d;
    if (!p->oflag) p->oflag = ctx->oflag_dev;
    return 0;
}
extern "C" int dz_k_gemm_g2(dz_ctx* ctx, const dz_convgemm_desc* d, int row_fragments, void* stream) {
    DzConvGemm p;
    if (int rc = gemm_gen_open("dz_k_gemm_g2", ctx, d, &p)) return rc;
    DzRangeScope range_scope(ctx->oflag_dev);
    return dz_launch_gemm_g2(p, row_fragments, (hipStream_t)stream);
}
extern "C" int dz_k_gemm_g3(dz_ctx* ctx, const dz_convgemm_desc* d, int row_fragments, void* stream) {
    DzConvGemm p;
    if (int rc = gemm_gen_open("dz_k_gemm_g3", ctx, d, &p)) return rc;
    DzRangeScope range_scope(ctx->oflag_dev);
    return dz_launch_gemm_g3(p, row_fragments, (hipStream_t)stream);
}
#endif
extern "C" int dz_k_mlp_head(dz_ctx* ctx, const void* xsplit, long long xplane, const void* w0split,
                             const void* w1split, const float* b0, const float* b1, const float* cw,
                             const float* cb, int rows, int frames, int classes, int speakers, int powerset,
                             float gamma, float beta, float* d_seg, float* d_weights, void* stream) {
    DZ_REQUIRE(ctx, "dz_k_mlp_head: NULL argument");
    DZ_HIP(hipSetDevice(ctx->device));
    DzRangeScope range_scope(ctx->oflag_dev);
    DzMlpHead m{};
    m.Xsplit = xsplit; m.xplane = xplane; m.W0split = w0split; m.W1split = w1split;
    m.b0 = b0; m.b1 = b1; m.cw = cw; m.cb = cb;
    m.rows = rows; m.F = frames; m.classes = classes; m.K = speakers; m.powerset = powerset;
    m.gamma = gamma; m.beta = beta; m.seg = d_seg; m.wout = d_weights;
    return dz_launch_mlp_head(m, (hipStream_t)stream);
}
extern "C" int dz_k_seg_head(dz_ctx* ctx, const float* m1, const float* cw, const float* cb, int batch,
                             int frames, int classes, int speakers, int powerset, float* d_seg, float gamma,
                             float beta, int normalize, float* d_weights, void* stream) {
    DZ_REQUIRE(ctx && m1 && cw && cb && d_seg, "dz_k_seg_head: NULL argument");
    DZ_HIP(hipSetDevice(ctx->device));
    return dz_launch_seg_head(m1, cw, cb, batch, frames, classes, speakers, powerset, d_seg, gamma, beta,
                              normalize, d_weights, (hipStream_t)stream);
}
extern "C" int dz_k_conv_pool(dz_ctx* ctx, const dz_convgemm_desc* d, void* stream) {
    DZ_REQUIRE(ctx && d, "dz_k_conv_pool: NULL argument");
    DZ_HIP(hipSetDevice(ctx->device));
    DzRangeScope range_scope(ctx->oflag_dev);
    DZ_REQUIRE(d->Wsplit && (d->Cin == 80 || d->Cin == 64), "dz_k_conv_pool: Wsplit is NULL or Cin is not 80 / 64");
    std::lock_guard<std::mutex> frag_lock(ctx->frag_mu);
    if (!ctx->convp_frag) DZ_HIP(hipMalloc(&ctx->convp_frag, (size_t)dz_conv_pool_wfrag_bytes(80)));
    if (ctx->convp_used && ctx->convp_user != (hipStream_t)stream) DZ_HIP(hipStreamSynchronize(ctx->convp_user));
    ctx->convp_user = (hipStream_t)stream; ctx->convp_used = true;
    int rc;
    if (!(dz_option(DZ_OPT_PACK_CACHE) && ctx->convp_src == d->Wsplit && ctx->convp_cin == d->Cin && ctx->convp_kpad == d->Kpad)) {
        if ((rc = dz_launch_conv_pool_wfrag(d->Cin, d->Wsplit, d->Kpad, ctx->convp_frag, (hipStream_t)stream))) return rc;
        ctx->convp_src = d->Wsplit; ctx->convp_cin = d->Cin; ctx->convp_kpad = d->Kpad;
    }
    return dz_launch_conv_pool(*d, (hipStream_t)stream, ctx->convp_frag);
}
#ifdef DZ_EXPERIMENTS
extern "C" int dz_k_conv_pool_debug(long long* d_stamps) {
    dz_conv_pool_dbg = d_stamps;
    return 0;
}
#endif
extern "C" int dz_k_convgemm_ntile(int t_out) { return dz_convgemm_ntile(t_out); }
extern "C" int dz_k_wave_stats(dz_ctx* ctx, const float* d_wave, long long stride, int batch,
                               int samples, float* d_stats, void* stream) {
    DZ_REQUIRE(ctx && d_stats, "dz_k_wave_stats: NULL argument");
    int rc;
    if ((rc = check_wave("dz_k_wave_stats", d_wave, stride, samples))) return rc;
    DZ_HIP(hipSetDevice(ctx->device));
    float* mom = nullptr;
    DZ_HIP(hipMalloc((void**)&mom, (size_t)batch * 2 * DZ_WS_G * sizeof(float)));
    rc = dz_launch_wave_stats(d_wave, stride, batch, samples, mom, (hipStream_t)stream);
    if (!rc) rc = dz_launch_wave_stats_combine(mom, batch, samples, d_stats, (hipStream_t)stream);
    (void)hipStreamSynchronize((hipStream_t)stream);
    (void)hipFree(mom);
    return rc;
}
extern "C" int dz_k_sinc_conv0(dz_ctx* ctx, const float* d_wave, long long stride, int batch,
                               int samples, const float* d_stats, float gamma, float beta,
                               const float* d_filt, float* d_y0, float* d_partials, void* stream) {
    DZ_REQUIRE(ctx && d_stats && d_filt && d_y0 && d_partials, "dz_k_sinc_conv0: NULL argument");
    int rc;
    if ((rc = check_wave("dz_k_sinc_conv0", d_wave, stride, samples))) return rc;
    const SincGeom g = sinc_geom(samples);
    DZ_REQUIRE(g.P0 > 0, "dz_k_sinc_conv0: %d samples is too short", samples);
    DZ_HIP(hipSetDevice(ctx->device));
    return dz_launch_sinc_conv0(d_wave, stride, batch, samples, d_stats, 0, gamma, beta, d_filt, d_y0,
                                g.P0, d_partials, g.nt0, (hipStream_t)stream);
}
extern "C" int dz_k_sinc_conv0_split(dz_ctx* ctx, const float* d_wave, long long stride, int batch,
                                     int samples, const float* d_stats, float gamma, float beta,
                                     const void* d_filt_split, float* d_y0, float* d_partials,
                                     void* stream) {
    DZ_REQUIRE(ctx && d_stats && d_filt_split && d_y0 && d_partials, "dz_k_sinc_conv0_split: NULL argument");
    int rc;
    if ((rc = check_wave("dz_k_sinc_conv0_split", d_wave, stride, samples))) return rc;
    const SincGeom g = sinc_geom(samples, true);
    DZ_REQUIRE(g.P0 > 0, "dz_k_sinc_conv0_split: %d samples is too short", samples);
    DZ_HIP(hipSetDevice(ctx->device));
    DzRangeScope range_scope(ctx->oflag_dev);
    std::lock_guard<std::mutex> frag_lock(ctx->frag_mu);
    if (!ctx->conv0_frag) DZ_HIP(hipMalloc(&ctx->conv0_frag, (size_t)dz_sinc_bank_frag_bytes()));
    if (ctx->conv0_used && ctx->conv0_user != (hipStream_t)stream) DZ_HIP(hipStreamSynchronize(ctx->conv0_user));
    ctx->conv0_user = (hipStream_t)stream; ctx->conv0_used = true;
    if (!(dz_option(DZ_OPT_PACK_CACHE) && ctx->conv0_src == d_filt_split)) {
        if ((rc = dz_launch_sinc_bank_frag(d_filt_split, ctx->conv0_frag, (hipStream_t)stream))) return rc;
        ctx->conv0_src = d_filt_split;
    }
    return dz_launch_sinc_conv0_split(d_wave, stride, batch, samples, d_stats, 0, gamma, beta,
                                      d_filt_split, d_y0, g.P0, d_partials, g.nt0, (hipStream_t)stream, ctx->conv0_frag);
}
extern "C" int dz_k_conv0_split_ntile(int samples) { return sinc_geom(samples, true).nt0; }
#ifdef DZ_EXPERIMENTS
extern "C" int dz_k_sinc_conv0_pair(dz_ctx* ctx, const float* d_wave, long long stride, int batch, int samples,
                                    const float* d_moments, const void* d_pair_planes, const float* d_pair_bsum,
                                    float gamma_seg, float gamma_emb, float* d_y0_seg, float* d_y0_emb,
                                    float* d_part_seg, float* d_part_emb, void* stream) {
    DZ_REQUIRE(ctx && d_moments && d_pair_planes && d_pair_bsum && d_y0_seg && d_y0_emb && d_part_seg && d_part_emb,
               "dz_k_sinc_conv0_pair: NULL argument");
    const SincGeom g = sinc_geom(samples, true);
    DZ_REQUIRE(batch >= 1 && g.F0 >= 3, "dz_k_sinc_conv0_pair: empty input");
    int rc;
    if ((rc = check_wave("dz_k_sinc_conv0_pair", d_wave, stride, samples))) return rc;
    DZ_HIP(hipSetDevice(ctx->device));
    DzRangeScope range_scope(ctx->oflag_dev);
    return dz_launch_sinc_conv0_pair(d_wave, stride, batch, samples, d_moments, d_pair_planes, d_pair_bsum, gamma_seg,
                                     gamma_emb, d_y0_seg, d_y0_emb, g.P0, d_part_seg, d_part_emb, g.nt0,
                                     (hipStream_t)stream);
}
#endif
extern "C" int dz_k_finalize_norm(dz_ctx* ctx, const float* d_partials, int batch, int ntile,
                                  int channels, int frames, const float* d_gamma,
                                  const float* d_beta, float* d_scale, float* d_shift,
                                  void* stream) {
    DZ_REQUIRE(ctx && d_partials && d_gamma && d_beta && d_scale && d_shift,
               "dz_k_finalize_norm: NULL argument");
    DZ_HIP(hipSetDevice(ctx->device));
    return dz_launch_finalize_norm(d_partials, batch, ntile, channels, frames, d_gamma, d_beta,
                                   d_scale, d_shift, (hipStream_t)stream);
}
extern "C" int dz_k_lstm(dz_ctx* ctx, const float* d_gx, const float* d_whh, float* d_hout,
                         int batch, int frames, void* stream) {
    DZ_REQUIRE(ctx && d_gx && d_whh && d_hout, "dz_k_lstm: NULL argument");
    DZ_REQUIRE(batch >= 1 && frames >= 1, "dz_k_lstm: empty input");
    DZ_HIP(hipSetDevice(ctx->device));
    return dz_launch_lstm(d_gx, d_whh, d_hout, nullptr, 0, batch, frames, 0, (hipStream_t)stream);
}
extern "C" int dz_k_lstm_planes(dz_ctx* ctx, const float* d_gx, const float* d_whh,
                                const void* d_whh_split, int variant, void* d_hsplit, long long hplane,
                                int batch, int frames, void* stream) {
    DZ_REQUIRE(ctx && d_gx && d_hsplit && (d_whh || d_whh_split), "dz_k_lstm_planes: NULL argument");
    DZ_REQUIRE(batch >= 1 && frames >= 1, "dz_k_lstm_planes: empty input");
    DZ_HIP(hipSetDevice(ctx->device));
    if (d_whh_split)
        return dz_launch_lstm_mfma(d_gx, d_whh_split, nullptr, d_hsplit, hplane, batch, frames, variant >= 3 ? 1 : 0,
                                   variant, (hipStream_t)stream);
    return dz_launch_lstm(d_gx, d_whh, nullptr, d_hsplit, hplane, batch, frames, 0, (hipStream_t)stream);
}
extern "C" int dz_k_lstm_mfma(dz_ctx* ctx, const float* d_gx, const void* d_whh_split, float* d_hout,
                              int batch, int frames, int unit_major, int variant, void* stream) {
    DZ_REQUIRE(ctx && d_gx && d_whh_split && d_hout, "dz_k_lstm_mfma: NULL argument");
    DZ_REQUIRE(batch >= 1 && frames >= 1, "dz_k_lstm_mfma: empty input");
    DZ_HIP(hipSetDevice(ctx->device));
    return dz_launch_lstm_mfma(d_gx, d_whh_split, d_hout, nullptr, 0, batch, frames, unit_major,
                               variant, (hipStream_t)stream);
}
extern "C" int dz_k_stats_pool(dz_ctx* ctx, const float* d_x, int frames, int channels, int ldx,
                               const float* d_weights, int weight_frames, int rows,
                               int rows_per_x, float* d_out, int ldo, void* stream) {
    DZ_REQUIRE(ctx && d_x && d_out, "dz_k_stats_pool: NULL argument");
    DZ_REQUIRE(rows >= 1 && rows_per_x >= 1 && frames >= 2, "dz_k_stats_pool: empty input");
    DZ_HIP(hipSetDevice(ctx->device));
    DZ_REQUIRE(!d_weights || weight_frames >= 2 || weight_frames <= -2, "dz_k_stats_pool: weight_frames %d", weight_frames);
    return dz_launch_stats_pool(d_x, (long long)frames * ldx, frames, channels, ldx, d_weights,
                                d_weights ? weight_frames : frames, rows, rows_per_x, d_out, ldo,
                                (hipStream_t)stream);
}
extern "C" int dz_k_powerset(dz_ctx* ctx, const float* d_logits, int rows, int classes,
                             int speakers, float* d_out, void* stream) {
    DZ_REQUIRE(ctx && d_logits && d_out, "dz_k_powerset: NULL argument");
    DZ_HIP(hipSetDevice(ctx->device));
    return dz_launch_powerset(d_logits, rows, classes, speakers, d_out, (hipStream_t)stream);
}
```

### diart_amd/csrc/xvec_api.hip

```cpp
#include "dz_sincnet.h"

struct dz_emb {
    dz_ctx* ctx;
    dz_emb_weights w;
    SincGeom g;
    int Bm, T[5];
    bool pre;
    const float* ext_stats;
    const float* cur_stats;
    int ext_conv0_B;
    char* arena;
    SincScratch ss;
    float *a, *b, *x5, *pooled, *parts, *ppart, *ps0;
    int pending_B;
    const float* pending_in;
};
static const int kTdnnTaps[5] = {5, 3, 3, 1, 1};
static const int kTdnnDil[5] = {1, 2, 3, 1, 1};
static const int kTdnnCin[5] = {64, 512, 512, 512, 512};
static const int kTdnnN[5] = {512, 512, 512, 512, 1536};
static const int kPoolLd = 3008;
static const int kMaxSpk = 8;
static const int kEmbSplit = 16;

extern "C" int dz_emb_frames_for(int num_samples) {
    const int f = sinc_geom(num_samples).P2 - 4 - 4 - 6;
    return f > 0 ? f : 0;
}

static void emb_carve(dz_emb* e, Arena& a) {
    e->ss.carve(a, e->g, e->Bm);
    e->a = a.take((size_t)e->Bm * e->g.P2 * 512);
    e->b = a.take((size_t)e->Bm * e->g.P2 * 512);
    e->x5 = a.take((size_t)e->Bm * e->g.P2 * 1536);
    e->pooled = a.take((size_t)e->Bm * kMaxSpk * kPoolLd);
    const int np = dz_pool_pieces(e->g.P2);
    e->ppart = a.take((size_t)e->Bm * np * 4 * 1536 * 2);
    e->ps0 = a.take((size_t)e->Bm * np * 4 * 2);
    e->parts = a.take((size_t)kEmbSplit * e->Bm * kMaxSpk * 512);
}

extern "C" int dz_emb_create(dz_ctx* ctx, const dz_emb_weights* w, int max_batch, int num_samples,
                             dz_emb** out) {
    DZ_REQUIRE(ctx && w && out, "dz_emb_create: NULL argument");
    DZ_REQUIRE(max_batch >= 1, "dz_emb_create: max_batch %d", max_batch);
    DZ_REQUIRE(w->dimension == 512, "dz_emb_create: dimension %d (only 512 is built)", w->dimension);
    const SincGeom g = sinc_geom(num_samples, w->sinc.filt_split != nullptr);
    DZ_REQUIRE(g.ok && g.P2 > 14, "dz_emb_create: %d samples is too short", num_samples);
    DZ_REQUIRE((w->sinc.w1_split != nullptr) == (w->sinc.w2_split != nullptr) &&
                   (w->sinc.w1_split != nullptr) == (w->tw_split[0] != nullptr),
               "dz_emb_create: the split planes of SincNet conv1 / conv2 and of tdnn1 must be all present "
               "or all absent (the consumer of the last SincNet stage finalises its InstanceNorm)");
    DZ_HIP(hipSetDevice(ctx->device));
    dz_emb* e = new (std::nothrow) dz_emb;
    DZ_REQUIRE(e != nullptr, "dz_emb_create: out of memory");
    e->ctx = ctx; e->w = *w; e->g = g; e->Bm = max_batch; e->arena = nullptr; e->ext_stats = nullptr; e->cur_stats = nullptr;
    e->ext_conv0_B = 0;
    e->pending_B = 0; e->pending_in = nullptr;
    e->pre = w->tw_split[0] && w->tw_split[1] && w->tw_split[2] &&
             w->tw_split[3] && w->tw_split[4];
    int t = g.P2;
    for (int i = 0; i < 5; ++i) {
        t -= (kTdnnTaps[i] - 1) * kTdnnDil[i];
        e->T[i] = t;
    }
    return sinc_handle_alloc("dz_emb_create", e, emb_carve, dz_emb_destroy, out);
}

extern "C" int dz_emb_destroy(dz_emb* emb) { return dz_handle_destroy(emb); }

extern "C" int dz_emb_use_wave_stats(dz_emb* emb, const float* d_moments) {
    DZ_REQUIRE(emb != nullptr, "dz_emb_use_wave_stats: NULL handle");
    emb->ext_stats = d_moments;
    return 0;
}

static DzGemm emb_tdnn(const dz_emb* e, int i, const void* wsplit, const float* in, bool in_planes, int B, float* out) {
    const long long rows = (long long)B * e->g.P2;
    const int cin = kTdnnCin[i], n = kTdnnN[i], K = cin * kTdnnTaps[i];
    const bool out_planes = e->pre && i < 4;
    const dz_layer L = {e->w.tw[i], e->w.tb[i], e->w.ts[i], e->w.th[i], wsplit};
    return DzGemm::dense(L, in, cin, rows, cin, out_planes ? nullptr : out, n, n, DZ_EPI_TDNN)
        .taps(kTdnnTaps[i], kTdnnDil[i], 0).padded((K + 31) / 32 * 32, n).xplanes(in_planes ? in : nullptr, rows * cin)
        .planes_out(out_planes ? out : nullptr, rows * n).prof(DZ_T_TDNN1 + i, B);
}
static DzGemm emb_tdnn5(const dz_emb* e, const float* in, int B, float* out) {
    return emb_tdnn(e, 4, e->w.tw_split[4], in, e->pre, B, out);
}

static int emb_frames(dz_emb* e, const float* d_wave, long long stride, int B, hipStream_t st) {
    const dz_emb_weights& w = e->w;
    int rc;
    const float* ext;
    bool pair;
    if ((rc = sinc_take_handoffs("dz_emb_frames", e, B, &ext, &pair))) return rc;
    const SincOut src = sinc_out_source(w.sinc, e->pre, w.tw0_split_kb);
    if ((rc = run_sincnet(w.sinc, e->g, e->ss, d_wave, stride, B, st, src, ext, pair))) return rc;
    e->cur_stats = ext ? ext : e->ss.stats;
    e->pending_B = 0;
    if (src == SINC_OUT_NORM_ON_LOAD) {
        const int P = e->g.P2;
        const dz_layer L = {w.tw[0], w.tb[0], w.ts[0], w.th[0], w.tw_split[0]};
        DzGemm g = DzGemm::conv1d(L, e->ss.y2, 64, B, P, 64, e->pre ? nullptr : e->a, 512, 512, DZ_EPI_TDNN).taps(5, 1, 0)
                       .padded(320, 512).planes_out(e->pre ? e->a : nullptr, (long long)B * P * 512).prof(DZ_T_TDNN1, B);
        rc = sinc_y2_norm(g, w.sinc, e->g, e->ss).run(st);
    } else {
        const bool planes = src == SINC_OUT_PLANES;
        rc = emb_tdnn(e, 0, planes ? w.tw0_split_kb : w.tw_split[0], e->ss.y2s, planes, B, e->a).run(st);
    }
    if (rc) return rc;
    const float* in = e->a;
    for (int i = 1; i < 4; ++i) {
        float* out = (i & 1) ? e->b : e->a;
        if ((rc = emb_tdnn(e, i, w.tw_split[i], in, e->pre, B, out).run(st))) return rc;
        in = out;
    }
    DzGemm g5 = emb_tdnn5(e, in, B, e->x5);
    if (e->pre && dz_option(DZ_OPT_POOL_FUSE) != 0 && e->g.P2 >= 128 && e->T[4] >= 2 && dz_gemm_pre_pool_ok(g5.p)) {
        e->pending_B = B;
        e->pending_in = in;
        return 0;
    }
    return g5.run(st);
}

static int emb_head(dz_emb* e, const float* d_weights, int Fw, int rows, int rows_per_x,
                    int normalize, float* d_out, hipStream_t st) {
    int rc;
    if (e->w.pool_nearest && d_weights) Fw = -Fw;
    const int nx = rows / rows_per_x, P = e->g.P2;
    bool pooled = false;
    if (e->pending_B > 0) {
        DZ_REQUIRE(nx == e->pending_B, "dz_emb_pool: %d chunks, but the frame features of %d are pending", nx,
                   e->pending_B);
        if (rows_per_x <= 4) {
            DzPoolFuse q;
            q.w = d_weights; q.Fw = Fw; q.K = rows_per_x; q.P = P; q.T = e->T[4]; q.np = dz_pool_pieces(P);
            q.part = e->ppart; q.s0 = e->ps0;
            if ((rc = emb_tdnn5(e, e->pending_in, nx, nullptr).run_pooled(q, st))) return rc;
            DzProfScope ps(DZ_T_POOL, nx);
            if ((rc = dz_launch_pool_combine(e->ppart, e->ps0, nx, rows_per_x, dz_pool_pieces(P), P, e->T[4], 1500, 1536,
                                             e->pooled, kPoolLd, st)))
                return rc;
            pooled = true;
        } else {
            if ((rc = emb_tdnn5(e, e->pending_in, nx, e->x5).run(st))) return rc;
            e->pending_B = 0;
        }
    }
    if (!pooled) {
        DzProfScope ps(DZ_T_POOL, nx);
        if ((rc = dz_launch_stats_pool(e->x5, (long long)P * 1536, e->T[4], 1500, 1536, d_weights, Fw, rows, rows_per_x,
                                       e->pooled, kPoolLd, st)))
            return rc;
    }
    const dz_layer lin = {e->w.emb_w, e->w.emb_b, nullptr, nullptr, nullptr};
    return dz_splitk_linear(lin, e->pooled, rows, kPoolLd, kPoolLd, 512, kEmbSplit, e->parts, normalize, d_out, st,
                            DZ_T_EMBLIN, DZ_T_L2, e->pre ? e->cur_stats : nullptr, rows_per_x);
}

struct EmbEntry {
    const char *who, *batch_fmt, *spk_fmt;
};
static int emb_open(const EmbEntry& en, dz_emb* e, bool have_args, int batch, int K, bool frames_ok, int weight_frames,
                    bool has_wave, const float* d_wave, long long wave_stride) {
    DZ_REQUIRE(e && have_args, "%s: NULL argument", en.who);
    DZ_REQUIRE(batch >= 1 && batch <= e->Bm, en.batch_fmt, en.who, batch, e->Bm);
    DZ_REQUIRE(K >= 1 && K <= kMaxSpk, en.spk_fmt, en.who, K, kMaxSpk);
    DZ_REQUIRE(frames_ok, "%s: weight_frames %d", en.who, weight_frames);
    if (has_wave)
        if (int rc = check_wave(en.who, d_wave, wave_stride, e->g.S)) return rc;
    DZ_HIP(hipSetDevice(e->ctx->device));
    return 0;
}

extern "C" int dz_emb_forward(dz_emb* e, const float* d_wave, long long wave_stride,
                              const float* d_weights, int n_rows, int weight_frames, float* d_out,
                              void* stream) {
    const EmbEntry en = {"dz_emb_forward", "%s: %d rows outside [1, %d]", ""};
    if (int rc = emb_open(en, e, d_out != nullptr, n_rows, 1, d_weights == nullptr || weight_frames >= 2, weight_frames,
                          true, d_wave, wave_stride))
        return rc;
    DzRangeScope range_scope(e->ctx->oflag_dev);
    hipStream_t st = (hipStream_t)stream;
    if (int rc = emb_frames(e, d_wave, wave_stride, n_rows, st)) return rc;
    return emb_head(e, d_weights, d_weights ? weight_frames : e->T[4], n_rows, 1, 0, d_out, st);
}

extern "C" int dz_emb_forward_multi(dz_emb* e, const float* d_wave, long long wave_stride,
                                    const float* d_weights, int batch, int num_speakers,
                                    int weight_frames, int normalize, float* d_out, void* stream) {
    const EmbEntry en = {"dz_emb_forward_multi", "%s: batch %d outside [1, %d]", "%s: %d speakers outside [1, %d]"};
    if (int rc = emb_open(en, e, d_out && d_weights, batch, num_speakers, weight_frames >= 2, weight_frames, true, d_wave,
                          wave_stride))
        return rc;
    DzRangeScope range_scope(e->ctx->oflag_dev);
    hipStream_t st = (hipStream_t)stream;
    if (int rc = emb_frames(e, d_wave, wave_stride, batch, st)) return rc;
    return emb_head(e, d_weights, weight_frames, batch * num_speakers, num_speakers, normalize,
                    d_out, st);
}

extern "C" int dz_emb_frames(dz_emb* e, const float* d_wave, long long wave_stride, int batch,
                             void* stream) {
    const EmbEntry en = {"dz_emb_frames", "%s: batch %d outside [1, %d]", ""};
    if (int rc = emb_open(en, e, true, batch, 1, true, 0, true, d_wave, wave_stride)) return rc;
    DzRangeScope range_scope(e->ctx->oflag_dev);
    return emb_frames(e, d_wave, wave_stride, batch, (hipStream_t)stream);
}
extern "C" int dz_emb_pool(dz_emb* e, const float* d_weights, int batch, int num_speakers,
                           int weight_frames, int normalize, float* d_out, void* stream) {
    const EmbEntry en = {"dz_emb_pool", "%s: batch %d outside [1, %d]", "%s: %d speakers"};
    if (int rc = emb_open(en, e, d_out && d_weights, batch, num_speakers, weight_frames >= 2, weight_frames, false, nullptr, 0))
        return rc;
    DzRangeScope range_scope(e->ctx->oflag_dev);
    return emb_head(e, d_weights, weight_frames, batch * num_speakers, num_speakers, normalize,
                    d_out, (hipStream_t)stream);
}

#ifdef DZ_EXPERIMENTS
extern "C" int dz_sinc_conv0_pair(dz_seg* seg_handle, dz_emb* emb, const float* d_wave, long long wave_stride, int batch,
                                  const float* d_moments, const void* d_pair_planes, const float* d_pair_bsum,
                                  void* stream) {
    DZ_REQUIRE(seg_handle && emb && d_moments && d_pair_planes && d_pair_bsum, "dz_sinc_conv0_pair: NULL argument");
    const SincFront seg = dz_seg_sinc_front(seg_handle);
    DZ_REQUIRE(seg.ctx == emb->ctx, "dz_sinc_conv0_pair: the two handles belong to different contexts");
    DZ_REQUIRE(batch >= 1 && batch <= seg.Bm && batch <= emb->Bm, "dz_sinc_conv0_pair: batch %d outside [1, %d]", batch,
               seg.Bm < emb->Bm ? seg.Bm : emb->Bm);
    DZ_REQUIRE(seg.g->S == emb->g.S && seg.g->nt0 == emb->g.nt0 && seg.g->P0 == emb->g.P0,
               "dz_sinc_conv0_pair: the handles were created for different window lengths");
    DZ_REQUIRE(seg.w->filt_split && emb->w.sinc.filt_split,
               "dz_sinc_conv0_pair: both networks must be in the split-f16 precision (the exact-f32 path keeps one "
               "launch per network)");
    int rc;
    if ((rc = check_wave("dz_sinc_conv0_pair", d_wave, wave_stride, seg.g->S))) return rc;
    DZ_HIP(hipSetDevice(seg.ctx->device));
    DzRangeScope range_scope(seg.ctx->oflag_dev);
    { DzProfScope ps(DZ_T_CONV0_PAIR, batch);
      if ((rc = dz_launch_sinc_conv0_pair(d_wave, wave_stride, batch, seg.g->S, d_moments, d_pair_planes, d_pair_bsum,
                                          seg.w->wav_gamma, emb->w.sinc.wav_gamma, seg.ss->y0, emb->ss.y0, seg.g->P0,
                                          seg.ss->part0, emb->ss.part0, seg.g->nt0, (hipStream_t)stream)))
          return rc; }
    *seg.ext_conv0_B = emb->ext_conv0_B = batch;
    return 0;
}
#endif
```

Measured before the change: 33830.

## Compute only valid rows per chunk in pre-split TDNN GEMMs via row map

Adds a row map so the pre-split GEMM and fused pool kernels compute only the valid output rows of each chunk, skipping the padded tail rows between chunks. A magic-number division maps compact row indices back to buffer rows for loads and stores. The TDNN layers of the x-vector embedding use it, and the pool fusion now pools compact chunks. The cost is extra index arithmetic per load and store, plus new kernel variants with stricter validity checks.

```diff
diff --git a/diart_amd/build.py b/diart_amd/build.py
--- a/diart_amd/build.py
+++ b/diart_amd/build.py
@@ -37,7 +37,7 @@
     hipcc = _hipcc()
     objdir = HERE / "build" / ("exp" if experiments else "ship")
     objdir.mkdir(parents=True, exist_ok=True)
-    headers = [CSRC / "dz_common.h", CSRC / "dz_embed.h", CSRC / "dz_sincnet.h", CSRC / "hostpool.h", CSRC / "tune_core.h", CSRC / "clu_core.h", HERE.parent / "include" / "diart_amd.h",
+    headers = [CSRC / "dz_common.h", CSRC / "dz_rowmap.h", CSRC / "dz_embed.h", CSRC / "dz_sincnet.h", CSRC / "hostpool.h", CSRC / "tune_core.h", CSRC / "clu_core.h", HERE.parent / "include" / "diart_amd.h",
                HERE.parent / "include" / "diart_amd_experiments.h"]
     flags = ["-O3", "-std=c++17", "-fPIC", f"--offload-arch={ARCH}", "-Wall", "-Wno-unused-function", f"-I{CSRC}"]
     sources, lib = list(SOURCES), LIB
diff --git a/diart_amd/csrc/dz_common.h b/diart_amd/csrc/dz_common.h
--- a/diart_amd/csrc/dz_common.h
+++ b/diart_amd/csrc/dz_common.h
@@ -5,6 +5,7 @@
 #include <stddef.h>
 #include <mutex>
 #include "../../include/diart_amd.h"
+#include "dz_rowmap.h"
 
 #ifdef DZ_EXPERIMENTS
 #include <stdlib.h>
@@ -287,7 +288,7 @@
 int dz_launch_conv_pool(const DzConvGemm& p, hipStream_t st, const void* wfrag = nullptr);
 int dz_conv_pool_wfrag_bytes(int Cin);
 int dz_launch_conv_pool_wfrag(int Cin, const void* wsplit, int Kpad, void* out, hipStream_t st);
-int dz_launch_gemm_pre(const DzConvGemm& p, hipStream_t st);
+int dz_launch_gemm_pre(const DzConvGemm& p, hipStream_t st, const DzRowMap& rm = DzRowMap{0, 0, 0u, 0});
 #ifdef DZ_EXPERIMENTS
 int dz_launch_gemm_g2(const DzConvGemm& p, int mt, hipStream_t st);
 int dz_g2_default_mt();
@@ -324,7 +325,8 @@
 };
 inline int dz_pool_pieces(int P) { return (P + 2 * 128 - 2) / 128; }
 bool dz_gemm_pre_pool_ok(const DzConvGemm& p);
-int dz_launch_gemm_pre_pool(const DzConvGemm& p, const DzPoolFuse& q, hipStream_t st);
+int dz_launch_gemm_pre_pool(const DzConvGemm& p, const DzPoolFuse& q, hipStream_t st,
+                            const DzRowMap& rm = DzRowMap{0, 0, 0u, 0});
 int dz_launch_pool_combine(const float* part, const float* s0, int nx, int K, int np, int P, int T, int C,
                            int Npad, float* out, int ldo, hipStream_t st);
 int dz_convgemm_ntile(int Tout);
diff --git a/diart_amd/csrc/dz_embed.h b/diart_amd/csrc/dz_embed.h
--- a/diart_amd/csrc/dz_embed.h
+++ b/diart_amd/csrc/dz_embed.h
@@ -13,6 +13,7 @@
     DzConvGemm p;
     const void *wsplit, *wfrag;
     int tag, units;
+    DzRowMap rm;
 
     static DzGemm dense(const dz_layer& L, const float* X, int ldx, long long rows, int Cin, float* Y, int ldy,
                         int Nstore, int epi) {
@@ -57,6 +58,11 @@
     }
     DzGemm& frag(const void* f) { wfrag = f; return *this; }
     DzGemm& tdev(const int* T) { p.Tdev = T; return *this; }
+    DzGemm& valid_rows(int Tv, int P) {
+        rm = dz_rowmap_make(Tv, P, p.Tin / P);
+        if (rm.Tv) p.Tout = p.Tstore = rm.rows / P * Tv;
+        return *this;
+    }
     DzGemm& prof(int t, int u) { tag = t; units = u; return *this; }
 
     int run(hipStream_t st) {
@@ -64,8 +70,9 @@
         if (p.Xsplit) {
             p.X = p.W = nullptr;
             p.Wsplit = wsplit;
-            return dz_launch_gemm_pre(p, st);
+            return dz_launch_gemm_pre(p, st, rm);
         }
+        DZ_REQUIRE(rm.Tv == 0, "DzGemm: valid_rows() asked of a layer that does not read pre-split activations");
         if (wsplit && p.ksplit <= 1) {
             p.Wsplit = wsplit;
             if (p.epi == DZ_EPI_POOL3)
@@ -80,7 +87,7 @@
         DzProfScope ps(tag, units);
         p.X = p.W = nullptr;
         p.Wsplit = wsplit;
-        return dz_launch_gemm_pre_pool(p, q, st);
+        return dz_launch_gemm_pre_pool(p, q, st, rm);
     }
 };
 
diff --git a/diart_amd/csrc/dz_rowmap.h b/diart_amd/csrc/dz_rowmap.h
--- /dev/null
+++ b/diart_amd/csrc/dz_rowmap.h
@@ -0,0 +1,32 @@
+#pragma once
+
+#if defined(__HIPCC__)
+#define DZ_ROWMAP_FN __host__ __device__ inline
+#else
+#define DZ_ROWMAP_FN inline
+#endif
+
+struct DzRowMap {
+    int Tv;
+    int P;
+    unsigned mul;
+    int rows;
+};
+
+inline DzRowMap dz_rowmap_make(int Tv, int P, int chunks) {
+    DzRowMap m = {0, 0, 0u, 0};
+    if (Tv <= 0 || Tv >= P) return m;
+    m.Tv = Tv;
+    m.P = P;
+    m.mul = Tv == 1 ? 0u : (unsigned)(((1ull << 32) + (unsigned)Tv - 1) / (unsigned)Tv);
+    m.rows = chunks * P;
+    return m;
+}
+inline bool dz_rowmap_exact(int Tv, long long rows) { return rows >= 0 && rows * Tv < (1ll << 32); }
+
+DZ_ROWMAP_FN unsigned dz_rowmap_chunk(const DzRowMap& m, unsigned r) {
+    return m.mul ? (unsigned)(((unsigned long long)r * m.mul) >> 32) : r;
+}
+DZ_ROWMAP_FN int dz_rowmap_row(const DzRowMap& m, int r) {
+    return r + (int)dz_rowmap_chunk(m, (unsigned)r) * (m.P - m.Tv);
+}
diff --git a/diart_amd/csrc/k_gemm_pre.hip b/diart_amd/csrc/k_gemm_pre.hip
--- a/diart_amd/csrc/k_gemm_pre.hip
+++ b/diart_amd/csrc/k_gemm_pre.hip
@@ -25,9 +25,14 @@
 constexpr int POOL_S0 = POOL_RED + 2 * 2 * 4 * BN * 4;
 constexpr size_t POOL_LDS = POOL_S0 + 8 * 8 * 2 * 4 + 8 * 2 * 4;
 
-template <int EPI, int MW, int MT, int NT, bool ILV = false, bool POOL = false>
+__device__ __forceinline__ int vr_voff(const DzRowMap& rm, const int r0, const int l) {
+    return dz_rowmap_row(rm, r0 + (l >> 2)) * 64 + (((l & 3) ^ ((l >> 4) & 3)) << 4);
+}
+
+template <int EPI, int MW, int MT, int NT, bool ILV = false, bool POOL = false, bool VR = false>
 __device__ __forceinline__ void gemm_pre_tile(const DzConvGemm& p, const int t0, const int n0, char* smem,
-                                              const int flags = 0, const DzPoolFuse* q = nullptr) {
+                                              const int flags = 0, const DzPoolFuse* q = nullptr,
+                                              const DzRowMap rm = DzRowMap{0, 0, 0u, 0}) {
     constexpr int PLANE_A = plane_a(MW), STAGE = stage_bytes(MW), PAR_OFF = POOL ? POOL_PAR : 2 * STAGE;
     static_assert(!POOL || (MW == 2 && MT == 2 && NT == 2), "pooled epilogue: 128 x 128 tiles only");
     const int tid = threadIdx.x;
@@ -50,6 +55,15 @@
     constexpr int vstep = 16 * 64;
     const int kb_bytes = prows * 64;
     const int dst0 = isB ? 2 * PLANE_A : 0, dplane = isB ? PLANE_B : PLANE_A;
+    int vmap[VR ? JMAX : 1];
+    if (VR) {
+#pragma unroll
+        for (int j = 0; j < (VR ? JMAX : 1); ++j) {
+            const int qj = rank + j * group, i = qj - (qj >= npc ? npc : 0);
+            vmap[j] = isB ? voff0 + i * vstep : vr_voff(rm, t0 + 16 * i, l);
+        }
+    }
+    const int* const vmap_p = vmap;
     auto issue = [&](int kt, int stage) {
         int cblk = kt, tap = 0;
         if (p.taps > 1) {
@@ -65,7 +79,7 @@
             const int lo = q >= npc, i = q - lo * npc;
             __builtin_amdgcn_raw_ptr_buffer_load_lds(lo ? rs_lo : rs_hi,
                 (__attribute__((address_space(3))) void*)(dst + lo * dplane + i * 1024), 16,
-                voff0 + i * vstep, soff, 0, 0);
+                VR ? vmap_p[VR ? j : 0] : voff0 + i * vstep, soff, 0, 0);
         }
     };
 
@@ -129,6 +143,13 @@
         const int r2 = w & 1;
         char* const dbase = smem + dst0 + r2 * 1024;
         const int vofs = voff0 + r2 * vstep;
+        int vofs4[VR ? 4 : 1];
+        if (VR) {
+#pragma unroll
+            for (int m = 0; m < (VR ? 4 : 1); ++m)
+                vofs4[m] = isB ? vofs + m * 2 * vstep : vr_voff(rm, t0 + 16 * (r2 + 2 * m), l);
+        }
+        const int* const vofs4_p = vofs4;
         int cblk = 0, tap = 0;
         const int tap_step = isB ? (p.Cin >> 5) * kb_bytes : p.dil * 64;
         auto advance = [&]() -> int {
@@ -144,7 +165,7 @@
             if (no_dma || (skip_a && tap != 0 && cblk > 0)) return;
             __builtin_amdgcn_raw_ptr_buffer_load_lds(lo ? rs_lo : rs_hi,
                 (__attribute__((address_space(3))) void*)(dbase + stage_next * STAGE + lo * dplane + (j & 3) * 2048), 16,
-                vofs + (j & 3) * 2 * vstep, soff_next, 0, 0);
+                VR ? vofs4_p[VR ? (j & 3) : 0] : vofs + (j & 3) * 2 * vstep, soff_next, 0, 0);
         };
         const char* sa0 = smem + (wm * 64) * 64;
         const char* sb0 = smem + 2 * PLANE_A + (wn * 64) * 64;
@@ -236,7 +257,7 @@
     if (POOL) __syncthreads();
     if constexpr (!POOL) {
         const bool whole = n0 + 64 * NT <= p.Nstore;
-        const long long ybytes = Yhi ? 2 * (long long)yrows * p.ldy : 4 * (long long)p.Tout * p.ldy;
+        const long long ybytes = Yhi ? 2 * (long long)yrows * p.ldy : 4 * (long long)(VR ? rm.rows : p.Tout) * p.ldy;
         if (whole && (Yhi != nullptr) != (p.Y != nullptr) && ybytes < (1ll << 31) && !(flags & 64)) {
             const unsigned nrec = __builtin_amdgcn_readfirstlane((unsigned)ybytes);
             const __amdgpu_buffer_rsrc_t r0 = __builtin_amdgcn_make_buffer_rsrc(Yhi ? (void*)Yhi : (void*)p.Y, 0, nrec, 0x00020000);
@@ -250,8 +271,9 @@
                 u32x2 ph = {0u, 0u}, pw = {0u, 0u};
 #pragma unroll
             for (int mt = 0; mt < MT; ++mt) {
-                const int t = t0 + wm * 32 * MT + mt * 32 + li;
-                const bool ok = t < p.Tout;
+                const int tc = t0 + wm * 32 * MT + mt * 32 + li;
+                const bool ok = tc < p.Tout;
+                const int t = VR ? dz_rowmap_row(rm, tc) : tc;
                 float am = 0.f;
                 const int vo = !ok ? (int)0x80000000 : KIND == 2 ? t * 64 + 16 * g : KIND == 1 ? t * 64 + 8 * g : (t * p.ldy + 4 * g) * 4;
 #pragma unroll
@@ -322,8 +344,9 @@
     }
 #pragma unroll
     for (int mt = 0; mt < MT; ++mt) {
-        const int t = t0 + wm * 32 * MT + mt * 32 + li;
-        const bool ok = t < p.Tout;
+        const int tc = t0 + wm * 32 * MT + mt * 32 + li;
+        const bool ok = tc < p.Tout;
+        const int t = VR ? dz_rowmap_row(rm, tc) : tc;
 #pragma unroll
         for (int nt = 0; nt < NT; ++nt)
 #pragma unroll
@@ -347,7 +370,7 @@
                     v[e] = x;
                 }
                 if (POOL) {
-                    if (!(flags & 16)) *reinterpret_cast<f32x4*>(yt + (t - t0) * YT_PITCH + nc) = v;
+                    if (!(flags & 16)) *reinterpret_cast<f32x4*>(yt + (tc - t0) * YT_PITCH + nc) = v;
                     continue;
                 }
                 const long long idx = (long long)t * p.ldy + n;
@@ -522,6 +545,27 @@
         gemm_pre_tile<EPI, 2, 1, 1>(p, mbig * BM + ms * 64, by * 64, smem);
     }
 }
+namespace vr {
+template <int EPI, bool ILV>
+__global__ __launch_bounds__(256, 2) void gemm_pre_kernel(DzConvGemm p, int mbig, int msmall, int flags, DzRowMap rm) {
+    extern __shared__ __attribute__((aligned(16))) char smem[];
+#ifndef DZ_EXPERIMENTS
+    flags = 0;
+#endif
+    const int gy = p.Npad / BN, L = blockIdx.x;
+    if (L < mbig * gy) {
+        int bx, by, bz;
+        dz_tile_map_lin(L, mbig, gy, 1, p.agroup, bx, by, bz);
+        gemm_pre_tile<EPI, 2, 2, 2, ILV, false, true>(p, bx * BM, by * BN, smem, flags, nullptr, rm);
+    } else {
+        const int Ls = L - mbig * gy, gys = 2 * gy;
+        const int xcd = Ls & 7, j = Ls >> 3;
+        const int ms = (j / gys) * 8 + xcd, by = j % gys;
+        if (ms >= msmall) return;
+        gemm_pre_tile<EPI, 2, 1, 1, false, false, true>(p, mbig * BM + ms * 64, by * 64, smem, 0, nullptr, rm);
+    }
+}
+}
 
 __global__ __launch_bounds__(256, 2) void gemm_pre_pool_kernel(DzConvGemm p, DzPoolFuse q, int gx, int flags) {
     extern __shared__ __attribute__((aligned(16))) char smem[];
@@ -533,6 +577,18 @@
 #endif
     gemm_pre_tile<DZ_EPI_TDNN, 2, 2, 2, true, true>(p, bx * BM, by * BN, smem, flags, &q);
 }
+namespace vr {
+__global__ __launch_bounds__(256, 2) void gemm_pre_pool_kernel(DzConvGemm p, DzPoolFuse q, int gx, int flags, DzRowMap rm) {
+    extern __shared__ __attribute__((aligned(16))) char smem[];
+    const int gy = p.Npad / BN;
+    int bx, by, bz;
+    dz_tile_map_lin(blockIdx.x, gx, gy, 1, p.agroup, bx, by, bz);
+#ifndef DZ_EXPERIMENTS
+    flags = 0;
+#endif
+    gemm_pre_tile<DZ_EPI_TDNN, 2, 2, 2, true, true, true>(p, bx * BM, by * BN, smem, flags, &q, rm);
+}
+}
 
 template <int EPI>
 __global__ __launch_bounds__(64 * 2 * MW_BIG) void gemm_pre_big_kernel(DzConvGemm p) {
@@ -583,9 +639,12 @@
 }
 
 template <int EPI>
-int launch(const DzConvGemm& p, hipStream_t st) {
-    static DzAttrOnce attr_ilv;
+int launch(const DzConvGemm& p, hipStream_t st, const DzRowMap& rm) {
+    static DzAttrOnce attr_ilv, attr_vr;
     DZ_HIP(attr_ilv.raise((const void*)gemm_pre_kernel<EPI, true>, (int)lds_bytes(2)));
+    if (rm.Tv) {
+        DZ_HIP(attr_vr.raise((const void*)vr::gemm_pre_kernel<EPI, true>, (int)lds_bytes(2)));
+    }
     const int gx = (p.Tout + BM - 1) / BM, gy = p.Npad / BN, slots = wg_slots();
 #ifdef DZ_EXPERIMENTS
     static DzAttrOnce attr_once, attr_big;
@@ -593,7 +652,7 @@
     {
         const int gxb = (p.Tout + 64 * MW_BIG - 1) / (64 * MW_BIG);
         const int mode = big_tiles_mode();
-        if (mode == 1 && gxb >= 8) {
+        if (mode == 1 && gxb >= 8 && !rm.Tv) {
             DZ_HIP(attr_big.raise((const void*)gemm_pre_big_kernel<EPI>, (int)lds_bytes(MW_BIG)));
             DZ_LAUNCH((gemm_pre_big_kernel<EPI>), dim3(gxb * gy), dim3(64 * 2 * MW_BIG), lds_bytes(MW_BIG), st, p);
             DZ_HIP(hipGetLastError());
@@ -611,10 +670,13 @@
     const int msmall = rows_left > 0 ? (rows_left + 63) / 64 : 0;
     const int nwg = mbig * gy + ((msmall + 7) / 8) * 8 * (2 * gy);
 #ifdef DZ_EXPERIMENTS
-    if (!interleaved_loop())
+    if (!interleaved_loop() && !rm.Tv)
         DZ_LAUNCH((gemm_pre_kernel<EPI, false>), dim3(nwg), dim3(256), lds_bytes(2), st, p, mbig, msmall, 0);
     else
 #endif
+    if (rm.Tv)
+        DZ_LAUNCH((vr::gemm_pre_kernel<EPI, true>), dim3(nwg), dim3(256), lds_bytes(2), st, p, mbig, msmall, dbg_flags(), rm);
+    else
         DZ_LAUNCH((gemm_pre_kernel<EPI, true>), dim3(nwg), dim3(256), lds_bytes(2), st, p, mbig, msmall, dbg_flags());
     DZ_HIP(hipGetLastError());
     return 0;
@@ -631,18 +693,35 @@
     return gen;
 }
 
+static int check_rowmap(const char* who, const DzConvGemm& p, const DzRowMap& rm) {
+    if (!rm.Tv) return 0;
+    DZ_REQUIRE(rm.Tv > 0 && rm.P > rm.Tv && rm.rows > 0 && rm.rows % rm.P == 0 && p.Tin == rm.rows &&
+                   p.Tout == rm.rows / rm.P * rm.Tv && rm.mul == dz_rowmap_make(rm.Tv, rm.P, 1).mul,
+               "%s: valid rows %d of pitch %d over %d buffer rows do not match Tin %d / Tout %d", who, rm.Tv, rm.P, rm.rows,
+               p.Tin, p.Tout);
+    DZ_REQUIRE(rm.Tv + (p.taps - 1) * p.dil <= rm.P, "%s: the taps of valid row %d reach past the chunk's %d rows", who,
+               rm.Tv - 1, rm.P);
+    DZ_REQUIRE(dz_rowmap_exact(rm.Tv, (long long)p.Tout + BM) &&
+                   p.xplane * 2 + ((long long)BM / rm.Tv + 2) * rm.P * 64 < (1ll << 31),
+               "%s: %d valid rows are beyond the row map's range", who, p.Tout);
+    return 0;
+}
+
 bool dz_gemm_pre_pool_ok(const DzConvGemm& p) {
     const int gx = (p.Tout + BM - 1) / BM, gy = p.Npad / BN;
     return 4 * gx * gy >= wg_slots();
 }
 
-int dz_launch_gemm_pre_pool(const DzConvGemm& p_in, const DzPoolFuse& q, hipStream_t st) {
+int dz_launch_gemm_pre_pool(const DzConvGemm& p_in, const DzPoolFuse& q, hipStream_t st, const DzRowMap& rm) {
     DzConvGemm p = p_in;
     if (!p.oflag) p.oflag = dz_cur_oflag;
     DZ_REQUIRE(p.Wsplit && p.Xsplit && q.part && q.s0, "gemm_pre_pool: NULL operand");
     DZ_REQUIRE(p.epi == DZ_EPI_TDNN && p.B == 1 && p.taps == 1 && p.K == p.Kpad && p.Cin % KT == 0 &&
-                   p.Npad % BN == 0 && p.Tout == p.Tin,
+                   p.Npad % BN == 0 && (rm.Tv || p.Tout == p.Tin),
                "gemm_pre_pool: built for the flattened 1 x 1 TDNN layer");
+    if (int rc = check_rowmap("gemm_pre_pool", p, rm)) return rc;
+    DZ_REQUIRE(!rm.Tv || (q.P == rm.Tv && q.T == rm.Tv),
+               "gemm_pre_pool: a valid-rows launch pools chunks of P = T = %d compact rows (got P %d, T %d)", rm.Tv, q.P, q.T);
     DZ_REQUIRE(q.np == dz_pool_pieces(q.P), "gemm_pre_pool: np must be dz_pool_pieces(P)");
     DZ_REQUIRE(q.K >= 1 && q.K <= 4 && q.P >= BM && q.T >= 2 && q.T <= q.P && p.Tout % q.P == 0 && (q.Fw >= 2 || q.Fw <= -2),
                "gemm_pre_pool: 1..4 speakers, chunk pitch >= 128 rows (got K %d, P %d, T %d)", q.K, q.P, q.T);
@@ -655,15 +734,20 @@
         return e && atoi(e) > 0 ? atoi(e) : 1;
     }();
     if (!p.agroup) p.agroup = pool_ag;
-    static DzAttrOnce attr_once;
-    DZ_HIP(attr_once.raise((const void*)gemm_pre_pool_kernel, (int)POOL_LDS));
+    static DzAttrOnce attr_once, attr_vr;
     const int gx = (p.Tout + BM - 1) / BM, gy = p.Npad / BN;
-    DZ_LAUNCH(gemm_pre_pool_kernel, dim3(gx * gy), dim3(256), POOL_LDS, st, p, q, gx, dbg_flags());
+    if (rm.Tv) {
+        DZ_HIP(attr_vr.raise((const void*)vr::gemm_pre_pool_kernel, (int)POOL_LDS));
+        DZ_LAUNCH(vr::gemm_pre_pool_kernel, dim3(gx * gy), dim3(256), POOL_LDS, st, p, q, gx, dbg_flags(), rm);
+    } else {
+        DZ_HIP(attr_once.raise((const void*)gemm_pre_pool_kernel, (int)POOL_LDS));
+        DZ_LAUNCH(gemm_pre_pool_kernel, dim3(gx * gy), dim3(256), POOL_LDS, st, p, q, gx, dbg_flags());
+    }
     DZ_HIP(hipGetLastError());
     return 0;
 }
 
-int dz_launch_gemm_pre(const DzConvGemm& p_in, hipStream_t st) {
+int dz_launch_gemm_pre(const DzConvGemm& p_in, hipStream_t st, const DzRowMap& rm) {
     DzConvGemm p = p_in;
     if (!p.oflag) p.oflag = dz_cur_oflag;
     DZ_REQUIRE(p.Wsplit != nullptr && p.Xsplit != nullptr,
@@ -673,20 +757,22 @@
     DZ_REQUIRE(p.K == p.Kpad && p.K == p.taps * p.Cin && p.Cin % KT == 0,
                "gemm_pre: K = taps * Cin without padding, Cin a multiple of 32");
     DZ_REQUIRE(p.Npad % BN == 0, "gemm_pre: Npad must be a multiple of 128");
-    DZ_REQUIRE(p.Tout > 0 && p.Tout == p.Tin - (p.taps - 1) * p.dil, "gemm_pre: Tout mismatch");
+    DZ_REQUIRE(p.Tout > 0 && (rm.Tv || p.Tout == p.Tin - (p.taps - 1) * p.dil), "gemm_pre: Tout mismatch");
+    if (int rc = check_rowmap("gemm_pre", p, rm)) return rc;
     DZ_REQUIRE(p.pad == 0 && p.X2 == nullptr && p.rowbias == nullptr && p.ksplit <= 1 && !p.norm_on_load,
                "gemm_pre: padding / second input / row bias / split-K / norm-on-load are not built here");
     DZ_REQUIRE(p.ldx > 0 && p.ldx % KT == 0 && p.xplane % p.ldx == 0 && p.xplane / p.ldx >= p.Tin,
                "gemm_pre: kb-major input planes need ldx %% 32 == 0 and xplane = rows * ldx with rows >= Tin");
     DZ_REQUIRE(p.xplane * 2 < (1ll << 31) && (long long)p.Npad * p.Kpad * 2 < (1ll << 31),
                "gemm_pre: operand plane exceeds the 2 GiB buffer-offset range");
-    DZ_REQUIRE(p.Ysplit == nullptr || (p.ldy > 0 && p.ldy % KT == 0 && p.yplane % p.ldy == 0 && p.yplane / p.ldy >= p.Tout &&
+    DZ_REQUIRE(p.Ysplit == nullptr || (p.ldy > 0 && p.ldy % KT == 0 && p.yplane % p.ldy == 0 &&
+                                       p.yplane / p.ldy >= (rm.Tv ? rm.rows : p.Tout) &&
                                        p.Npad <= p.ldy && p.yplane * 2 < (1ll << 31)),
                "gemm_pre: kb-major output planes need ldy %% 32 == 0, yplane = rows * ldy with rows >= Tout, Npad <= ldy");
     DZ_REQUIRE(p.Y == nullptr || (p.ldy % 4 == 0 && ((uintptr_t)p.Y & 15) == 0),
                "gemm_pre: f32 output needs ldy a multiple of 4 and a 16-byte aligned base");
 #ifdef DZ_EXPERIMENTS
-    if (dz_gemm_gen() >= 2 && 4 * ((p.Tout + BM - 1) / BM) * (p.Npad / BN) >= wg_slots()) {
+    if (!rm.Tv && dz_gemm_gen() >= 2 && 4 * ((p.Tout + BM - 1) / BM) * (p.Npad / BN) >= wg_slots()) {
         static const int g3_min_k = [] {
             const char* e = dz_exp_env("DZ_G3_MINK");
             return e ? atoi(e) : 1024;
@@ -699,10 +785,10 @@
     }
 #endif
     switch (p.epi) {
-        case DZ_EPI_BIAS: return launch<DZ_EPI_BIAS>(p, st);
-        case DZ_EPI_BIAS_LEAKY: return launch<DZ_EPI_BIAS_LEAKY>(p, st);
-        case DZ_EPI_TDNN: return launch<DZ_EPI_TDNN>(p, st);
-        case DZ_EPI_RELU_BN: return launch<DZ_EPI_RELU_BN>(p, st);
+        case DZ_EPI_BIAS: return launch<DZ_EPI_BIAS>(p, st, rm);
+        case DZ_EPI_BIAS_LEAKY: return launch<DZ_EPI_BIAS_LEAKY>(p, st, rm);
+        case DZ_EPI_TDNN: return launch<DZ_EPI_TDNN>(p, st, rm);
+        case DZ_EPI_RELU_BN: return launch<DZ_EPI_RELU_BN>(p, st, rm);
     }
     dz_set_error("gemm_pre: epilogue %d is not built on the pre-split path", p.epi);
     return 2;
diff --git a/diart_amd/csrc/kernel_api.hip b/diart_amd/csrc/kernel_api.hip
--- a/diart_amd/csrc/kernel_api.hip
+++ b/diart_amd/csrc/kernel_api.hip
@@ -21,6 +21,17 @@
     DZ_REQUIRE(ctx && d, "dz_k_gemm_pre: NULL argument");
     DZ_HIP(hipSetDevice(ctx->device));
     DzRangeScope range_scope(ctx->oflag_dev);
+    if (d->B > 1) {
+        DZ_REQUIRE(d->ldx > 0 && d->ldy > 0 && d->xbs > 0 && d->xbs % d->ldx == 0 && d->ybs == d->xbs / d->ldx * d->ldy &&
+                       d->xbs / d->ldx >= d->Tin && d->xbs / d->ldx * d->B < (1ll << 31) && d->Tout > 0 &&
+                       d->Tout == d->Tin - (d->taps - 1) * d->dil,
+                   "dz_k_gemm_pre: B = %d chunks need xbs / ldx = ybs / ldy >= Tin rows per chunk and Tout = Tin - (taps - 1) dil",
+                   d->B);
+        const int P = (int)(d->xbs / d->ldx);
+        DzConvGemm p = *d;
+        p.B = 1; p.Tin = d->B * P; p.Tout = p.Tstore = d->B * d->Tout;
+        return dz_launch_gemm_pre(p, (hipStream_t)stream, dz_rowmap_make(d->Tout, P, d->B));
+    }
     return dz_launch_gemm_pre(*d, (hipStream_t)stream);
 }
 #ifdef DZ_EXPERIMENTS
diff --git a/diart_amd/csrc/xvec_api.hip b/diart_amd/csrc/xvec_api.hip
--- a/diart_amd/csrc/xvec_api.hip
+++ b/diart_amd/csrc/xvec_api.hip
@@ -82,7 +82,8 @@
     const dz_layer L = {e->w.tw[i], e->w.tb[i], e->w.ts[i], e->w.th[i], wsplit};
     return DzGemm::dense(L, in, cin, rows, cin, out_planes ? nullptr : out, n, n, DZ_EPI_TDNN)
         .taps(kTdnnTaps[i], kTdnnDil[i], 0).padded((K + 31) / 32 * 32, n).xplanes(in_planes ? in : nullptr, rows * cin)
-        .planes_out(out_planes ? out : nullptr, rows * n).prof(DZ_T_TDNN1 + i, B);
+        .planes_out(out_planes ? out : nullptr, rows * n).valid_rows(in_planes ? e->T[i] : e->g.P2, e->g.P2)
+        .prof(DZ_T_TDNN1 + i, B);
 }
 static DzGemm emb_tdnn5(const dz_emb* e, const float* in, int B, float* out) {
     return emb_tdnn(e, 4, e->w.tw_split[4], in, e->pre, B, out);
@@ -116,7 +117,7 @@
         in = out;
     }
     DzGemm g5 = emb_tdnn5(e, in, B, e->x5);
-    if (e->pre && dz_option(DZ_OPT_POOL_FUSE) != 0 && e->g.P2 >= 128 && e->T[4] >= 2 && dz_gemm_pre_pool_ok(g5.p)) {
+    if (e->pre && dz_option(DZ_OPT_POOL_FUSE) != 0 && e->T[4] >= 128 && dz_gemm_pre_pool_ok(g5.p)) {
         e->pending_B = B;
         e->pending_in = in;
         return 0;
@@ -135,11 +136,13 @@
                    e->pending_B);
         if (rows_per_x <= 4) {
             DzPoolFuse q;
-            q.w = d_weights; q.Fw = Fw; q.K = rows_per_x; q.P = P; q.T = e->T[4]; q.np = dz_pool_pieces(P);
+            DzGemm g5 = emb_tdnn5(e, e->pending_in, nx, nullptr);
+            const int Pc = g5.rm.Tv ? g5.rm.Tv : P;
+            q.w = d_weights; q.Fw = Fw; q.K = rows_per_x; q.P = Pc; q.T = e->T[4]; q.np = dz_pool_pieces(Pc);
             q.part = e->ppart; q.s0 = e->ps0;
-            if ((rc = emb_tdnn5(e, e->pending_in, nx, nullptr).run_pooled(q, st))) return rc;
+            if ((rc = g5.run_pooled(q, st))) return rc;
             DzProfScope ps(DZ_T_POOL, nx);
-            if ((rc = dz_launch_pool_combine(e->ppart, e->ps0, nx, rows_per_x, dz_pool_pieces(P), P, e->T[4], 1500, 1536,
+            if ((rc = dz_launch_pool_combine(e->ppart, e->ps0, nx, rows_per_x, q.np, Pc, e->T[4], 1500, 1536,
                                              e->pooled, kPoolLd, st)))
                 return rc;
             pooled = true;
```

Measured after the change: 33130. 0.979x the previous value.
